# medical-genomics-group/VAMPomi

Measured on AMD Instinct MI355X. Metric: VAMP iterations/s (+ achieved HBM GB/s of the A/A^T kernels), higher is better.
Workload: dtype f64

## Files before the change

### include/vampomi.h

```cpp
#ifndef VAMPOMI_H
#define VAMPOMI_H

#include <stddef.h>
#include <stdint.h>

#ifdef __cplusplus
extern "C" {
#endif

#define VAMPOMI_ABI_VERSION 3
#define VAMPOMI_MAX_L 64
#define VAMPOMI_MAX_C 64
#define VAMPOMI_MAX_SEGMENTS 64
#define VAMPOMI_UNIQUE_ID_BYTES 128

typedef enum {
    VAMPOMI_OK = 0,
    VAMPOMI_ERR_ARG = 1,
    VAMPOMI_ERR_HIP = 2,
    VAMPOMI_ERR_RCCL = 3,
    VAMPOMI_ERR_IO = 4,
    VAMPOMI_ERR_NAN_PHEN = 5,
    VAMPOMI_ERR_STATE = 6,
    VAMPOMI_ERR_OOM = 7,
// ... 171 lines not shown
    double bytes_total;
    double flops_total;
    int64_t timed;
    double ms_timed;
} vampomi_kernel_stat;

typedef struct {
    vampomi_kernel_stat ax;
    vampomi_kernel_stat atx;
    vampomi_kernel_stat ax_k[4];
    vampomi_kernel_stat atx_k[4];
    int64_t a_passes_exec;
    int64_t host_syncs;
    vampomi_kernel_stat loo;
    vampomi_kernel_stat op;
    vampomi_kernel_stat op_k[4];
    vampomi_kernel_stat coll;
} vampomi_stats;

vampomi_status vampomi_set_timing(vampomi_ctx* ctx, int on);
vampomi_status vampomi_get_stats(vampomi_ctx* ctx, vampomi_stats* out);
vampomi_status vampomi_reset_stats(vampomi_ctx* ctx);

vampomi_status vampomi_dev_set_variant(vampomi_ctx* ctx, int which, int variant);
vampomi_status vampomi_dev_prestep_counts(const vampomi_ctx* ctx, int64_t* made, int64_t* used);
vampomi_status vampomi_dev_time_pass(vampomi_ctx* ctx, int which, int K, int reps, double* avg_ms);
vampomi_status vampomi_dev_read_ceiling(vampomi_ctx* ctx, int reps, double* us_med, double* bytes, int* variant);
vampomi_status vampomi_dev_kernel_name(const vampomi_ctx* ctx, int which, int K, int mode, char* out, int cap);
vampomi_status vampomi_dev_ax_plan(int64_t N, int64_t M, int cus, int variant, int K, int* T, int* TR, int* S,
                                   int* grid, int* nslots, char* name, int cap);
vampomi_status vampomi_dev_op_plan(int64_t N, int64_t M, int cus, int variant, int K, int* T, int* S, int* TR,
                                   int* grid, int64_t* nslots, char* name, int cap);
vampomi_status vampomi_dev_op_lds(int64_t N, int64_t M, int cus, int variant, int K, int64_t* out);
vampomi_status vampomi_dev_op_timestamps(vampomi_ctx* ctx, unsigned long long* out, int cap, int* n);
vampomi_status vampomi_dev_mem_plan(int64_t N, int64_t Mt, int nranks, int rank, int cus, int probit, int writer,
                                    int64_t* bytes);
vampomi_status vampomi_dev_mem_plan_storage(int64_t N, int64_t Mt, int nranks, int rank, int cus, int probit,
                                            int writer, int storage, int64_t* bytes);
vampomi_status vampomi_dev_op_apply(vampomi_ctx* ctx, int K, const double* ar, const double* qo, const double* p,
                                    const double* z, const double* beta, double diag, double tau, double gam2,
                                    double* d, double* ad, double* dp);

#ifdef __cplusplus
}
#endif
#endif
```

### vampomi_amd/__init__.py

```python
from __future__ import annotations

import ctypes as C
from dataclasses import dataclass, field
from typing import Optional, Sequence

import numpy as np

from ._lib import (CLI_PATH, GEN_GAUSS, GEN_METH, LIB_PATH, MAX_L, MEM_DEVICE, MEM_HOST, NA_FATAL, NA_MEAN, NA_PASS,
                   STORE_F32, STORE_F64, STORE_U16, UNIQUE_ID_BYTES, Params, Result, ShardDesc, Stats, VampomiError,
                   check, load)

__all__ = ["Data", "Vamp", "VampOptions", "divide_work", "comm_unique_id", "phen_rows", "phen_rows_common", "read_labels", "adjust_basis", "VampomiError", "LIB_PATH", "CLI_PATH",
           "GEN_GAUSS", "GEN_METH", "STORE_F64", "STORE_F32", "STORE_U16", "load"]

_STORAGE = {"f64": STORE_F64, "f32": STORE_F32, "u16": STORE_U16}
_METH_NA = {"pass": NA_PASS, "fatal": NA_FATAL, "mean": NA_MEAN}


def _dp(a: np.ndarray):
    return a.ctypes.data_as(C.c_void_p)


def divide_work(Mt: int, nranks: int, rank: int):
    M, S, Mm = C.c_int64(), C.c_int64(), C.c_int64()
# ... 416 lines not shown
        pr = np.ascontiguousarray(probs, dtype=np.float64)
        va = np.ascontiguousarray(vars_scaled, dtype=np.float64)
        x1 = np.zeros(max(self.M, 1))
        x1d = np.zeros(max(self.M, 1))
        s = C.c_double()
        check(self._lib.vampomi_denoise(self.ctx, _dp(r1), gam1, _dp(pr), _dp(va), L, _dp(x1), _dp(x1d),
                                        C.byref(s), MEM_HOST))
        return x1[: self.M], x1d[: self.M], s.value

    def kernel_name(self, which: int, K: int, mode: int = 0) -> str:
        buf = C.create_string_buffer(256)
        check(self._lib.vampomi_dev_kernel_name(self.ctx, which, K, mode, buf, 256))
        return buf.value.decode()

    def op_apply(self, ar, p, diag: float, tau: float, gam2: float, z=None, qo=None, beta=None):
        ar = np.ascontiguousarray(np.atleast_2d(ar), dtype=np.float64)
        p = np.ascontiguousarray(np.atleast_2d(p), dtype=np.float64)
        K = ar.shape[0]
        if ar.shape != (K, self.N) or p.shape != (K, self.M):
            raise ValueError("ar must be K x N and p K x M")
        fz = z is not None
        if fz:
            z = np.ascontiguousarray(np.atleast_2d(z), dtype=np.float64)
            qo = np.ascontiguousarray(np.atleast_2d(qo), dtype=np.float64)
            beta = np.ascontiguousarray(beta, dtype=np.float64)
        d = np.zeros((K, max(self.M, 1)))
        ad = np.zeros((K, self.N))
        dp = np.zeros(K)
        check(self._lib.vampomi_dev_op_apply(self.ctx, K, _dp(ar), _dp(qo) if fz else None, _dp(p),
                                             _dp(z) if fz else None, _dp(beta) if fz else None, diag, tau, gam2,
                                             _dp(d), _dp(ad), _dp(dp)))
        return d[:, : self.M], ad, dp

    def read_ceiling(self, reps: int = 9) -> dict:
        us, nb, var = C.c_double(), C.c_double(), C.c_int()
        check(self._lib.vampomi_dev_read_ceiling(self.ctx, int(reps), C.byref(us), C.byref(nb), C.byref(var)))
        return {"us_med": us.value, "bytes": nb.value, "GBs": nb.value / (us.value * 1e-6) / 1e9,
                "variant": ("lockstep 8-wave workgroups, one per CU", "1 MiB chunk per wave")[var.value]}

    def set_variant(self, which: int, variant: int):
        check(self._lib.vampomi_dev_set_variant(self.ctx, which, variant))

    def prestep_counts(self) -> tuple:
        made, used = C.c_int64(), C.c_int64()
        check(self._lib.vampomi_dev_prestep_counts(self.ctx, C.byref(made), C.byref(used)))
        return made.value, used.value

    def all_ok(self, local_ok: bool) -> bool:
        out = C.c_int()
        check(self._lib.vampomi_all_ok(self.ctx, 1 if local_ok else 0, C.byref(out)))
        return bool(out.value)

    def comm_abort(self):
        check(self._lib.vampomi_comm_abort(self.ctx))

    def set_timing(self, on: bool = True, period: int = 1):
        check(self._lib.vampomi_set_timing(self.ctx, (max(1, int(period)) if on else 0)))

    def stats(self) -> Stats:
        s = Stats()
        check(self._lib.vampomi_get_stats(self.ctx, C.byref(s)))
        return s

    def reset_stats(self):
        check(self._lib.vampomi_reset_stats(self.ctx))

# ... 146 lines not shown
```

### vampomi_amd/_lib.py

```python
from __future__ import annotations

import ctypes as C
import os

try:
    import torch
except Exception:
    torch = None

HERE = os.path.dirname(os.path.abspath(__file__))
LIB_PATH = os.environ.get("VAMPOMI_LIB") or os.path.join(HERE, "lib", "libvampomi.so")
CLI_PATH = os.path.join(HERE, "bin", "main_meth.exe")

MAX_L = 64
MAX_C = 64
UNIQUE_ID_BYTES = 128
MEM_HOST, MEM_DEVICE = 0, 1
GEN_GAUSS, GEN_METH = 0, 1
STORE_F64, STORE_F32, STORE_U16 = 0, 1, 16
NA_PASS, NA_FATAL, NA_MEAN = 0, 1, 2

STATUS = {
    0: "OK", 1: "ERR_ARG", 2: "ERR_HIP", 3: "ERR_RCCL", 4: "ERR_IO",
    5: "ERR_NAN_PHEN", 6: "ERR_STATE", 7: "ERR_OOM", 8: "ERR_MODEL",
# ... 121 lines not shown
    "vampomi_read_covariates": (C.c_int, [_P, C.c_char_p, C.c_int]),
    "vampomi_set_covariates": (C.c_int, [_P, _P, C.c_int, C.c_int64, C.c_int]),
    "vampomi_get_covariates": (C.c_int, [_P, _P]),
    "vampomi_cov_eval": (C.c_int, [_P, _P, _P, _P, _P, C.POINTER(C.c_double), C.c_int]),
    "vampomi_newton_cov": (C.c_int, [_P, _P, _P, _P, C.POINTER(C.c_int), _P, _P, C.c_int]),
    "vampomi_get_cov_eff": (C.c_int, [_P, _P]),
    "vampomi_get_probit_state": (C.c_int, [_P, _P, C.POINTER(C.c_double)]),
    "vampomi_denoise": (C.c_int, [_P, _P, C.c_double, _P, _P, C.c_int, _P, _P, C.POINTER(C.c_double), C.c_int]),
    "vampomi_params_default": (None, [C.POINTER(Params)]),
    "vampomi_infere": (C.c_int, [_P, C.POINTER(Params), C.POINTER(Result)]),
    "vampomi_vamp_begin": (C.c_int, [_P, C.POINTER(Params), C.POINTER(Result)]),
    "vampomi_vamp_step": (C.c_int, [_P, C.POINTER(C.c_int)]),
    "vampomi_step_phases": (C.c_int, [_P, C.POINTER(C.c_double), C.POINTER(C.c_double)]),
    "vampomi_vamp_end": (C.c_int, [_P]),
    "vampomi_set_timing": (C.c_int, [_P, C.c_int]),
    "vampomi_get_stats": (C.c_int, [_P, C.POINTER(Stats)]),
    "vampomi_reset_stats": (C.c_int, [_P]),
    "vampomi_dev_set_variant": (C.c_int, [_P, C.c_int, C.c_int]),
    "vampomi_dev_prestep_counts": (C.c_int, [_P, C.POINTER(C.c_int64), C.POINTER(C.c_int64)]),
    "vampomi_dev_time_pass": (C.c_int, [_P, C.c_int, C.c_int, C.c_int, C.POINTER(C.c_double)]),
    "vampomi_dev_read_ceiling": (C.c_int, [_P, C.c_int, C.POINTER(C.c_double), C.POINTER(C.c_double),
                                           C.POINTER(C.c_int)]),
    "vampomi_dev_kernel_name": (C.c_int, [_P, C.c_int, C.c_int, C.c_int, C.c_char_p, C.c_int]),
    "vampomi_dev_mem_plan": (C.c_int, [C.c_int64, C.c_int64, C.c_int, C.c_int, C.c_int, C.c_int, C.c_int, _P]),
    "vampomi_dev_mem_plan_storage": (C.c_int, [C.c_int64, C.c_int64, C.c_int, C.c_int, C.c_int, C.c_int, C.c_int,
                                               C.c_int, _P]),
    "vampomi_dev_ax_plan": (C.c_int, [C.c_int64, C.c_int64, C.c_int, C.c_int, C.c_int, _P, _P, _P, _P, _P, C.c_char_p,
                                      C.c_int]),
    "vampomi_dev_op_plan": (C.c_int, [C.c_int64, C.c_int64, C.c_int, C.c_int, C.c_int, _P, _P, _P, _P, _P, C.c_char_p,
                                      C.c_int]),
    "vampomi_dev_op_lds": (C.c_int, [C.c_int64, C.c_int64, C.c_int, C.c_int, C.c_int, _P]),
    "vampomi_dev_op_apply": (C.c_int, [_P, C.c_int, _P, _P, _P, _P, _P, C.c_double, C.c_double, C.c_double, _P, _P,
                                       _P]),
    "vampomi_dev_op_timestamps": (C.c_int, [_P, _P, C.c_int, C.POINTER(C.c_int)]),
    "vampomi_all_ok": (C.c_int, [_P, C.c_int, C.POINTER(C.c_int)]),
    "vampomi_comm_abort": (C.c_int, [_P]),
}

_lib = None


def load() -> C.CDLL:
    global _lib
    if _lib is None:
        if not os.path.exists(LIB_PATH):
            raise ImportError(f"{LIB_PATH} not built: run `python -m vampomi_amd.build`")
        lib = C.CDLL(LIB_PATH, mode=C.RTLD_GLOBAL)
        other = bool(os.environ.get("VAMPOMI_LIB"))
        for name, (res, args) in SIGNATURES.items():
            if other and not hasattr(lib, name):
                continue
            f = getattr(lib, name)
            f.restype = res
            f.argtypes = args
        _lib = lib
    return _lib


def check(status: int) -> None:
    if status != 0:
        msg = load().vampomi_last_error()
        raise VampomiError(status, msg.decode() if msg else "")
```

### vampomi_amd/csrc/atax_team.hip

```cpp
#include <hip/hip_ext.h>

#include <algorithm>
#include <cstdio>
#include <mutex>
#include <string>
#include <type_traits>

#include "kdev.h"

namespace vk {

typedef unsigned int v4u __attribute__((ext_vector_type(4)));
typedef unsigned int v2u __attribute__((ext_vector_type(2)));

#ifndef TM_FMA
#define TM_FMA 1
#endif
#ifndef TM_SAFE
#define TM_SAFE 0
#endif
#ifndef TM_TS
#define TM_TS 0
#endif
#ifndef TM_TEAMS_BY_XCD
// ... 143 lines not shown
__device__ __forceinline__ XE tm_ld1(__amdgpu_buffer_rsrc_t rs, int off) {
    if constexpr (sizeof(XE) == 8)
        return __builtin_bit_cast(double, __builtin_amdgcn_raw_buffer_load_b64(rs, off, 0, 2));
    else if constexpr (sizeof(XE) == 4)
        return __builtin_bit_cast(float, __builtin_amdgcn_raw_buffer_load_b32(rs, off, 0, 2));
    else
        return (uint16_t)__builtin_amdgcn_raw_buffer_load_b16(rs, off, 0, 2);
}

template <class Tp>
__device__ __forceinline__ Tp* tm_chk(Tp* p, const void* lo, const void* hi, unsigned code, unsigned* err) {
#if TM_SAFE
    if ((const char*)p < (const char*)lo || (const char*)p >= (const char*)hi) {
        __hip_atomic_fetch_or(err, 1u | (code << 1), __ATOMIC_RELAXED, __HIP_MEMORY_SCOPE_SYSTEM);
        return (Tp*)lo;
    }
#endif
    return p;
}

template <int K>
struct TmSlots {
    const double* ar[K];
    const double* p[K];
    double* d[K];
    double* sraw[K];
    double diag[K], tau[K], gam2[K];
};
template <int K>
__device__ __forceinline__ TmSlots<K> tm_slots(const OpArgs& a, int alt) {
    TmSlots<K> s;
#pragma unroll
    for (int k = 0; k < K; ++k) {
        int idx = k == alt ? kOpMaxK : k;
        asm volatile("" : "+s"(idx));
        const OpAlt::Slot& t = a.alt.tab[idx];
        s.ar[k] = t.ar;
        s.p[k] = t.p;
        s.d[k] = t.d;
        s.sraw[k] = t.sraw;
        s.diag[k] = t.diag;
        s.tau[k] = t.tau;
        s.gam2[k] = t.gam2;
    }
    return s;
}

template <int K, int S, int F, int L, int P, bool COMM, int E, bool FMA, int KP, class XE>
__device__ __forceinline__ void atax_team_body(const XE* __restrict__ X, int64_t ld, int64_t N, int64_t M,
                                               const double* __restrict__ mave, const double* __restrict__ msig,
                                               const OpArgs& a, int T, int TR, int ilv,
                                               const int* __restrict__ gate) {
    extern __shared__ __attribute__((aligned(16))) double lds[];
    double* s_beta = lds;
    if (a.fold.on) {
        double& s_go = lds[kOpMaxK];
        if (threadIdx.x == 0) {
            CgState cs = *a.fold.src;
            double r[3 * kMaxRhs];
#pragma unroll
            for (int q = 0; q < 3 * kMaxRhs; ++q) r[q] = q < 3 * cs.K ? a.fold.red[q] : 0.0;
            const bool ran = cg_decide_into(cs, r, a.fold.it, a.fold.mask);
            if (blockIdx.x == 0) {
                *a.fold.dst = cs;
                cg_publish(cs, ran, a.fold.it, a.fold.mirror, a.fold.flag, a.fold.seq, a.fold.pack);
            }
            s_go = cs.any ? 1.0 : 0.0;
#pragma unroll
            for (int k = 0; k < kOpMaxK; ++k) s_beta[k] = cs.beta[k];
        }
        __syncthreads();
        if (s_go == 0.0) return;
    } else if (gate && !*gate) {
        return;
    }
    const double* beta = a.fold.on ? s_beta : a.beta;
    static_assert(K + KP <= kMaxRhs, "partial slots per team");
    int fuse = a.fuse, alt = -1;
    if constexpr (KP == 0) {
        if (a.alt.cs && !a.fold.on) alt = cg_pre_slot(a.alt.cs->active, K, *a.alt.done == a.alt.token);
        if (alt >= 0) fuse &= ~(1 << alt);
    }
#if TM_TS
    const unsigned long long ts0 = __builtin_amdgcn_s_memrealtime();
#endif
    const int dbg = TM_ABL ? TM_ABL : (TM_DBG || !COMM) ? a.dbg : 0;
    constexpr int CW = COMM ? 7 : 8;
    constexpr int RS = tm_rows_per_step(COMM, E);
    static_assert(E == 1 || E == 2, "doubles per lane per load");
    constexpr int RING = F + L + 1;
    static_assert(COMM || L == 0, "without a hand-off the column is finished in its own step");
    static_assert(!COMM || (P >= 1 && P <= L), "polls in flight");
    static_assert(!COMM || P < RING, "a poll's slot is consumed before it is reissued");
    const int wave = threadIdx.x >> 6, lane = threadIdx.x & 63;
    const int g = blockIdx.x >> 3;
    const int member = g % T;
    const int nteams = gridDim.x / T;
#if TM_TEAMS_BY_XCD
    const int team = g / T + (nteams >> 3) * (int)(blockIdx.x & 7);
#else
    const int team = (blockIdx.x & 7) + 8 * (g / T);
#endif
    const int64_t cs = ilv ? nteams : 1;
    const int64_t mb = ilv ? team : (int64_t)team * M / nteams;
    const int n = (int)(ilv ? (M - team + nteams - 1) / nteams : (int64_t)(team + 1) * M / nteams - mb);
    const int64_t nmax = (M + nteams - 1) / nteams;
    const int64_t gwords = (M + gridDim.x) * kOpMaxK * T * 2;
    const int64_t r0 = (int64_t)member * TR;
    const int nrows = (int)(N - r0 < TR ? N - r0 : TR);
    constexpr bool QFULL = tm_qfull(K, S, COMM, E);
    const TmLds lay = tm_lds(K, S, COMM, E, TR < N ? TR : N);
    const int QS = (int)lay.qs;
    double* q_lds = lds + lay.q;
    double* s_part = lds + lay.part;
    double* s_tot = lds + lay.tot;
    const int jb = 64 * E * wave + E * lane;
    constexpr int XB = (int)sizeof(XE);
    const int nbytes = (E == 2 ? (nrows + 1) & ~1 : nrows) * XB;

    if (COMM && wave == CW) {
        const TmSlots<K> sl = tm_slots<K>(a, alt);
        const int nq = K * T;
        unsigned long long* xg = a.xg + (int64_t)team * nmax * nq * 2;
        unsigned long long* dummy = a.xg + gwords + (int64_t)blockIdx.x * 2 * K;
        const bool qv = (lane >> 5) < K && (lane & 31) < T;
        const int ql2 = qv ? 2 * ((lane >> 5) * T + (lane & 31)) : 0;
        const int nq2 = 2 * nq;
        const int csi = (int)cs;
        const unsigned tag = a.tag;
        const double* scp = msig;
#pragma unroll
        for (int k = 0; k < K; ++k) {
            if (lane == 1 + k) scp = sl.p[k];
            if (lane == 1 + K + k && ((fuse >> k) & 1)) scp = a.z.p[k];
        }
        scp += mb;
        double bk[K], dpacc[K];
#pragma unroll
        for (int k = 0; k < K; ++k) {
            bk[k] = ((fuse >> k) & 1) ? beta[k] : 0.0;
            dpacc[k] = 0.0;
        }
        v4u pl[RING];
        v2u ps[RING];
        bool dead = false;
        unsigned nslow = 0, nspin = 0;
        if (n > 0) {
            bool l2 = false;
            {
                unsigned long long* hdr = a.xg + gwords + (int64_t)gridDim.x * 2 * kOpMaxK + (int64_t)team * T;
                unsigned xcc;
                asm volatile("s_getreg_b32 %0, hwreg(HW_REG_XCC_ID)" : "=s"(xcc));
                xcc &= 0xf;
                if (lane == 0)
                    __hip_atomic_store(hdr + member, ((unsigned long long)tag << 32) | xcc, __ATOMIC_RELAXED,
                                       __HIP_MEMORY_SCOPE_AGENT);
                unsigned long long h = 0;
                for (unsigned spins = 0;; ++spins) {
                    h = lane < T ? __hip_atomic_load(hdr + lane, __ATOMIC_RELAXED, __HIP_MEMORY_SCOPE_AGENT)
                                 : ((unsigned long long)tag << 32) | xcc;
                    if (__all((unsigned)(h >> 32) == tag)) break;
                    if (spins >= kTmMaxSpins) {
                        dead = true;
                        if (lane == 0) __hip_atomic_store(a.err, 1u, __ATOMIC_RELAXED, __HIP_MEMORY_SCOPE_SYSTEM);
                        break;
                    }
                    __builtin_amdgcn_s_sleep(2);
                }
                l2 = !dead && __all((unsigned)h == xcc);
                if (dbg & 32) l2 = false;
            }
            for (int base = -F; base - L < n; base += RING) {
#pragma unroll
                for (int i = 0; i < RING; ++i) {
                    const int m = base + i;
                    if (dbg & 4096) {
                        __syncthreads();
                        continue;
                    }
                    const int ci = m - L + P, cf = m - L;
                    const int cic = ci < 0 ? 0 : ci < n ? ci : n - 1;
                    tm_load8(ps[(i + RING - L + P) % RING], scp + cic * csi);
                    tm_poll(pl[(i + RING - L + P) % RING], xg + (cic * nq2 + ql2));
                    v4u& g = pl[(i + RING - L) % RING];
                    v2u& sc = ps[(i + RING - L) % RING];
                    if (!(dbg & 1)) tm_wait2<3 * P>(g, sc);
                    if (cf >= 0 && cf < n) {
                        if (!(__all(g.y == tag && g.w == tag) || dead || (dbg & 1))) {
#pragma unroll 1
                            for (unsigned spins = 0;; ++spins) {
                                if (dbg & 64) {
                                    nslow += spins == 0;
                                    nspin++;
                                }
                                if (spins >= kTmMaxSpins) {
                                    dead = true;
                                    if (lane == 0) __hip_atomic_store(a.err, 1u, __ATOMIC_RELAXED, __HIP_MEMORY_SCOPE_SYSTEM);
                                    break;
                                }
                                __builtin_amdgcn_s_sleep(2);
                                tm_poll(g, tm_chk(xg + ((int64_t)cf * nq2 + ql2), a.xg, a.xg + gwords, 64, a.err));
                                tm_wait<0>(g);
                                if (__all(g.y == tag && g.w == tag)) break;
                            }
                        }
                        double v = qv ? __builtin_bit_cast(double, ((unsigned long long)g.z << 32) | g.x) : 0.0;
                        if (dbg & 512) {
                            for (int o = T >> 1; o > 0; o >>= 1) v += __shfl_xor(v, o, 64);
                        } else if (!(dbg & 256)) {
                            v = group_sum<32>(v);
                        }
                        const double scv = __builtin_bit_cast(double, ((unsigned long long)sc.y << 32) | sc.x);
                        const double sg = readlane_d(scv, 0);
                        const bool own = (cf & (T - 1)) == member;
                        const int64_t mg = mb + cf * csi;
                        double tsc[K], dval[K], pdir[K];
#pragma unroll
                        for (int k = 0; k < K; ++k) {
                            double t = sg * readlane_d(v, 32 * k);
                            t *= a.scale;
                            double p = readlane_d(scv, 1 + k);
                            if ((fuse >> k) & 1) p = readlane_d(scv, 1 + K + k) + bk[k] * p;
                            double val = t * sl.tau[k];
                            val += sl.gam2[k] * p;
                            tsc[k] = t;
                            dval[k] = val;
                            pdir[k] = p;
                        }
#pragma unroll
                        for (int k = 0; k < K; ++k)
                            if (lane == 0) s_tot[(cf & 1) * K + k] = (dbg & 128) ? 0.0 : sg * dval[k];
                        if (own) {
#pragma unroll
                            for (int k = 0; k < K; ++k) {
                                if (lane == 0 && !(dbg & 1024)) {
                                    if (a.sraw.p[0]) sl.sraw[k][mg] = tsc[k];
                                    *tm_chk(sl.d[k] + mg, sl.d[k], sl.d[k] + M, 128, a.err) = dval[k];
                                }
                                dpacc[k] += dval[k] * pdir[k];
                            }
                        }
                    }
                    __syncthreads();
                    if (lane < K && !(dbg & 2)) {
                        const bool real = m >= 0 && m < n;
                        double v = 0.0;
                        if (real) v = tree_sum<CW>(s_part + (m & 1) * CW * K + lane, K);
                        const unsigned long long u = __builtin_bit_cast(unsigned long long, v);
                        const v4u gr = {(unsigned)u, tag, (unsigned)(u >> 32), tag};
                        unsigned long long* dst =
                            tm_chk(real ? xg + ((int64_t)m * nq2 + (lane * T + member) * 2) : dummy + 2 * lane, a.xg,
                                   a.xg + gwords + (int64_t)gridDim.x * 2 * kOpMaxK, 512, a.err);
                        if (l2)
                            tm_publish_l2(dst, gr);
                        else
                            tm_publish(dst, gr);
                    }
                }
            }
#pragma unroll
            for (int s = 0; s < RING; ++s) tm_wait2<0>(pl[s], ps[s]);
            if ((dbg & 64) && lane == 0) {
                __hip_atomic_fetch_add(a.err + 1, nslow, __ATOMIC_RELAXED, __HIP_MEMORY_SCOPE_SYSTEM);
                __hip_atomic_fetch_add(a.err + 2, nspin, __ATOMIC_RELAXED, __HIP_MEMORY_SCOPE_SYSTEM);
                __hip_atomic_fetch_add(a.err + 3, (unsigned)n, __ATOMIC_RELAXED, __HIP_MEMORY_SCOPE_SYSTEM);
            }
        }
        if (lane == 0) {
#pragma unroll
            for (int k = 0; k < K; ++k) red_put(a.ro, (int64_t)blockIdx.x * K + k, dpacc[k]);
        }
        asm volatile("s_waitcnt vmcnt(0)" ::: "memory");
        __syncthreads();
        return;
    }

    const TmSlots<K> sl = tm_slots<K>(a, alt);
#pragma unroll
    for (int s = 0; s < S; ++s) {
        const int jl = RS * s + jb;
        if (jl >= QS) continue;
#pragma unroll
        for (int k = 0; k < K; ++k) {
#pragma unroll
            for (int h = 0; h < E; ++h) {
                double q = 0.0;
                if (jl + h < nrows) {
                    const int64_t j = r0 + jl + h;
                    q = sl.ar[k][j] / sl.diag[k];
                    if ((fuse >> k) & 1) q = q + beta[k] * a.qo.p[k][j];
                }
                q_lds[k * QS + jl + h] = q;
            }
        }
    }
    double bk[K];
#pragma unroll
    for (int k = 0; k < K; ++k) bk[k] = ((fuse >> k) & 1) ? beta[k] : 0.0;
    const double* pkp = mave;
    if (lane == 1) pkp = msig;
#pragma unroll
    for (int k = 0; k < K; ++k) {
        if (lane == 2 + k) pkp = sl.p[k];
        if (lane == 2 + K + k && ((fuse >> k) & 1)) pkp = a.z.p[k];
    }
#pragma unroll
    for (int k = 0; k < KP; ++k)
        if (lane == 2 + 2 * K + k) pkp = a.px.p[k];
    pkp += mb;
    bool valid[S];
#pragma unroll
    for (int s = 0; s < S; ++s) valid[s] = RS * s + jb < nrows;
    double acc[K][S][E];
#pragma unroll
    for (int k = 0; k < K; ++k)
#pragma unroll
        for (int s = 0; s < S; ++s)
#pragma unroll
            for (int e = 0; e < E; ++e) acc[k][s][e] = 0.0;
    double dpacc[K];
#pragma unroll
    for (int k = 0; k < K; ++k) dpacc[k] = 0.0;
    constexpr int KPA = KP > 0 ? KP : 1;
    double accp[KPA][S][E];
#pragma unroll
    for (int k = 0; k < KPA; ++k)
#pragma unroll
        for (int s = 0; s < S; ++s)
#pragma unroll
            for (int e = 0; e < E; ++e) accp[k][s][e] = 0.0;

    constexpr bool NW = XB < 8;
    typedef typename std::conditional<NW, XE, float>::type XW;
    double xr[NW ? 1 : RING][S][E];
    XW xw[NW ? RING : 1][S][E];
    double pk[RING];
    const char* xtile = reinterpret_cast<const char*>(X + mb * ld + r0);
// ... 46 lines not shown
            }
            if constexpr (KP > 0) {
#pragma unroll
                for (int k = 0; k < KP; ++k)
#pragma unroll
                    for (int e = 0; e < E; ++e) {
                        if constexpr (FMA)
                            accp[k][s][e] = __builtin_fma(dx[e], cp[k], accp[k][s][e]);
                        else
                            accp[k][s][e] += dx[e] * cp[k];
                    }
            }
#pragma unroll
            for (int k = 0; k < K; ++k) {
                if ((TM_DBG || TM_ABL) && (dbg & 2048)) {
                    q[k][0] = 0.5;
                    q[k][E - 1] = 0.25;
                } else if constexpr (E == 2) {
                    const v2d qq = *reinterpret_cast<const v2d*>(q_lds + k * QS + jq);
                    q[k][0] = qq.x;
                    q[k][E - 1] = qq.y;
                } else {
                    q[k][0] = q_lds[k * QS + jq];
                }
#pragma unroll
                for (int e = 0; e < E; ++e) {
                    if constexpr (FMA)
                        v[k] = __builtin_fma(dx[e], q[k][e], v[k]);
                    else
                        v[k] += dx[e] * q[k][e];
                }
            }
        }
        if (K == 2) {
            double r0, r1;
            swap32(v[0], v[K - 1], r0, r1);
            double keep = r0 + r1;
            if (dbg & 512) {
                for (int o = 16; o > 0; o >>= 1) keep += __shfl_xor(keep, o, 64);
            } else if (!(dbg & 4)) {
                keep = group_sum<32>(keep);
            }
            if ((lane & 31) == 0) s_part[(par * CW + wave) * K + (lane >> 5)] = keep;
        } else {
            if (!(dbg & 4)) v[0] = group_sum<64>(v[0]);
            if (lane == 0) s_part[(par * CW + wave) * K] = v[0];
        }
    };
    auto finish = [&](int slot, int m, const double (&tot)[K]) {
        double cc[K];
        if constexpr (COMM) {
#pragma unroll
            for (int k = 0; k < K; ++k) cc[k] = tot[k];
        } else {
            const double sg = readlane_d(pk[slot], 1);
            const bool own = (m % T) == member;
            const int64_t mg = mb + m * cs;
#pragma unroll
            for (int k = 0; k < K; ++k) {
                double t = sg * tot[k];
                t *= a.scale;
                double p = readlane_d(pk[slot], 2 + k);
                if ((fuse >> k) & 1) p = readlane_d(pk[slot], 2 + K + k) + bk[k] * p;
                double val = t * sl.tau[k];
                val += sl.gam2[k] * p;
                if (own) {
                    if (threadIdx.x == 0) {
                        if (a.sraw.p[0]) sl.sraw[k][mg] = t;
                        sl.d[k][mg] = val;
                    }
                    dpacc[k] += val * p;
                }
                cc[k] = sg * val;
            }
        }
        const double mu = NW ? readlane_d(pk[slot], 0) : 0.0;
#pragma unroll
        for (int s = 0; s < S; ++s) {
            if (dbg & 8) break;
            const double me_ = QFULL || valid[s] ? mu : 0.0;
#pragma unroll
            for (int k = 0; k < K; ++k)
#pragma unroll
                for (int e = 0; e < E; ++e) {
                    double dx;
                    if constexpr (NW)
                        dx = widen1(xw[slot][s][e]) - me_;
                    else
                        dx = xr[slot][s][e];
                    if constexpr (FMA)
                        acc[k][s][e] = __builtin_fma(dx, cc[k], acc[k][s][e]);
                    else
                        acc[k][s][e] += dx * cc[k];
                }
        }
    };
// ... 18 lines not shown
                            double t = 0.0;
#pragma unroll
                            for (int w = 0; w < CW; ++w) t += s_part[((m & 1) * CW + w) * K + k];
                            tot[k] = t;
                        }
                    }
                    finish((i + RING - L) % RING, cf, tot);
                }
            }
        }
    }
    double* dst = a.part + (int64_t)team * kMaxRhs * ld + r0;
#pragma unroll
    for (int s = 0; s < S; ++s) {
        const int jl = RS * s + jb;
        if (jl >= nrows) continue;
#pragma unroll
        for (int k = 0; k < K; ++k)
#pragma unroll
            for (int e = 0; e < E; ++e)
                if (jl + e < nrows) dst[(int64_t)k * ld + jl + e] = acc[k][s][e];
        if constexpr (KP > 0) {
#pragma unroll
            for (int k = 0; k < KP; ++k)
#pragma unroll
                for (int e = 0; e < E; ++e)
                    if (jl + e < nrows) dst[(int64_t)(K + k) * ld + jl + e] = accp[k][s][e];
        }
    }
    if constexpr (COMM) {
        __syncthreads();
    } else if (threadIdx.x == 0) {
#pragma unroll
        for (int k = 0; k < K; ++k) red_put(a.ro, (int64_t)blockIdx.x * K + k, dpacc[k]);
    }
    if (wave == 0) ticket_sum_blocks<K>(a.ro);
#if TM_TS
    if (a.ts && threadIdx.x == 0) {
        unsigned xcc, hw;
        asm volatile("s_getreg_b32 %0, hwreg(HW_REG_XCC_ID)" : "=s"(xcc));
        asm volatile("s_getreg_b32 %0, hwreg(HW_REG_HW_ID)" : "=s"(hw));
        unsigned long long* t = a.ts + 4 * (int64_t)blockIdx.x;
        t[0] = ts0;
        t[1] = __builtin_amdgcn_s_memrealtime();
        t[2] = xcc;
        t[3] = hw;
    }
#endif
}

template <int K, int S, int F, int L, int P, bool COMM, int E, bool FMA>
__global__ __launch_bounds__(kTmThreads) void atax_team_kernel(const double* __restrict__ X, int64_t ld, int64_t N,
                                                               int64_t M, const double* __restrict__ mave,
                                                               const double* __restrict__ msig, OpArgs a, int T,
                                                               int TR, int ilv, const int* __restrict__ gate) {
    atax_team_body<K, S, F, L, P, COMM, E, FMA, 0>(X, ld, N, M, mave, msig, a, T, TR, ilv, gate);
}

template <int K, int S, int F, int L, int P, bool COMM, int E, bool FMA>
__global__ __launch_bounds__(kTmThreads) void atax_team_kernel_f32(const float* __restrict__ X, int64_t ld,
                                                                   int64_t N, int64_t M,
                                                                   const double* __restrict__ mave,
                                                                   const double* __restrict__ msig, OpArgs a, int T,
                                                                   int TR, int ilv, const int* __restrict__ gate) {
    atax_team_body<K, S, F, L, P, COMM, E, FMA, 0>(X, ld, N, M, mave, msig, a, T, TR, ilv, gate);
}

template <int K, int S, int F, int L, int P, bool COMM, int E, bool FMA>
__global__ __launch_bounds__(kTmThreads) void atax_team_kernel_u16(const uint16_t* __restrict__ X, int64_t ld,
// ... 167 lines not shown
static int tm_S(int64_t rows, bool comm, int E) {
    const int rs = tm_rows_per_step(comm, E);
    return (int)((rows + rs - 1) / rs);
}

bool team_plan(int64_t N, int64_t M, int cus, int T, int cfg, OpPlan* out) {
    if (cfg < 0 || cfg >= kTmNCfg || N < 1) return false;
    const TmCfg& c = kTmCfg[cfg];
    if ((T == 1) == c.comm) return false;
    if (T < 1 || T > kTmMaxT || (T & (T - 1))) return false;
    const int grid = (cus / (8 * T)) * 8 * T;
    if (grid < T) return false;
    int64_t TR = N;
    if (T > 1) {
        TR = c.E == 2 ? ((N + T - 1) / T + 127) / 128 * 128 : (N + T - 1) / T;
        if ((int64_t)(T - 1) * TR >= N) return false;
    }
    const int S = tm_S(TR, c.comm, c.E);
    if (S > c.maxS) return false;
    for (int K = 1; K <= kOpMaxK; ++K)
        if (tm_lds(K, S, c.comm, c.E, std::min<int64_t>(TR, N)).words * 8 > kTmLdsMaxBytes) return false;
    OpPlan p{};
    p.grid = grid;
    p.S = S;
    p.T = T;
    p.TR = (int)TR;
    p.cfg = cfg;
    p.nslots = grid / T;
    (void)M;
    *out = p;
    return true;
}

bool team_lds_layout(const OpPlan& pl, int64_t N, int K, int64_t out[6]) {
    if (pl.T < 1 || pl.cfg < 0 || pl.cfg >= kTmNCfg || K < 1 || K > kOpMaxK || N < 1) return false;
    const TmCfg& c = kTmCfg[pl.cfg];
    const TmLds l = tm_lds(K, pl.S, c.comm, c.E, std::min<int64_t>(pl.TR, N));
    out[0] = kTmLdsHead;
    out[1] = l.q;
    out[2] = l.qs;
    out[3] = l.part;
    out[4] = l.tot;
    out[5] = l.words;
    return true;
}

template <int K, int S, int C, bool PL, class XE>
static hipError_t launch_tm_e(const Shard& s, const OpPlan& pl, const OpArgs& a, hipStream_t st, const Timing& tm,
                              const int* gate, int* occ) {
    constexpr TmCfg c = kTmCfg[C];
    static_assert(!PL || K == 1, "the head-start kernel has one operator system");
    constexpr bool F32 = sizeof(XE) == 4, U16 = sizeof(XE) == 2;
    void (*kern)(const XE*, int64_t, int64_t, int64_t, const double*, const double*, OpArgs, int, int, int,
                 const int*);
    if constexpr (PL && U16)
        kern = atax_team_plain_kernel_u16<S, c.F, c.L, c.P, c.comm, c.E, (bool)TM_FMA>;
    else if constexpr (U16)
        kern = atax_team_kernel_u16<K, S, c.F, c.L, c.P, c.comm, c.E, (bool)TM_FMA>;
    else if constexpr (PL && F32)
        kern = atax_team_plain_kernel_f32<S, c.F, c.L, c.P, c.comm, c.E, (bool)TM_FMA>;
    else if constexpr (PL)
        kern = atax_team_plain_kernel<S, c.F, c.L, c.P, c.comm, c.E, (bool)TM_FMA>;
    else if constexpr (F32)
        kern = atax_team_kernel_f32<K, S, c.F, c.L, c.P, c.comm, c.E, (bool)TM_FMA>;
    else
        kern = atax_team_kernel<K, S, c.F, c.L, c.P, c.comm, c.E, (bool)TM_FMA>;
    const size_t lds = (size_t)tm_lds(K, S, c.comm, c.E, std::min<int64_t>(pl.TR, s.N)).words * sizeof(double);
    if (lds > (size_t)kTmLdsMaxBytes) return hipErrorInvalidValue;
    static std::atomic<unsigned long long> allowed{0};
    if (const hipError_t e = lds_allow(reinterpret_cast<const void*>(kern), allowed, (int)kTmLdsMaxBytes))
        return e;
    if (occ) {
        if (hipOccupancyMaxActiveBlocksPerMultiprocessor(occ, kern, kTmThreads, lds) != hipSuccess) *occ = 0;
        return hipSuccess;
    }
    hipExtLaunchKernelGGL(kern, dim3(pl.grid), dim3(kTmThreads), lds, st, tm.start, tm.stop, 0,
                          static_cast<const XE*>(s.X), s.ld, s.N, s.M, s.mave, s.msig, a, pl.T, pl.TR, c.ilv ? 1 : 0,
                          gate);
    return hipSuccess;
}

template <int K, int S, int C, bool PL>
static hipError_t launch_tm(const Shard& s, const OpPlan& pl, const OpArgs& a, hipStream_t st, const Timing& tm,
                            const int* gate, int* occ) {
    if (s.u16) return launch_tm_e<K, S, C, PL, uint16_t>(s, pl, a, st, tm, gate, occ);
    if (s.f32) return launch_tm_e<K, S, C, PL, float>(s, pl, a, st, tm, gate, occ);
    return launch_tm_e<K, S, C, PL, double>(s, pl, a, st, tm, gate, occ);
}

static constexpr int tm_plain_maxS(int cfg) {
    return cfg == 0 ? 8 : cfg == 2 ? 3 : cfg == 3 ? 4 : cfg == 4 ? 5 : 0;
}

template <int K, int C, int S, bool PL>
static hipError_t launch_tm_if(const Shard& s, const OpPlan& pl, const OpArgs& a, hipStream_t st, const Timing& tm,
                               const int* gate, int* occ) {
    if constexpr (S <= (PL ? tm_plain_maxS(C) : kTmCfg[C].maxS))
        return launch_tm<K, S, C, PL>(s, pl, a, st, tm, gate, occ);
    return hipErrorInvalidValue;
}

template <int K, int C, bool PL>
static hipError_t launch_tm_s(int S, const Shard& s, const OpPlan& pl, const OpArgs& a, hipStream_t st,
                        const Timing& tm, const int* gate, int* occ) {
    switch (S) {
        case 1: return launch_tm_if<K, C, 1, PL>(s, pl, a, st, tm, gate, occ);
        case 2: return launch_tm_if<K, C, 2, PL>(s, pl, a, st, tm, gate, occ);
        case 3: return launch_tm_if<K, C, 3, PL>(s, pl, a, st, tm, gate, occ);
        case 4: return launch_tm_if<K, C, 4, PL>(s, pl, a, st, tm, gate, occ);
        case 5: return launch_tm_if<K, C, 5, PL>(s, pl, a, st, tm, gate, occ);
        case 6: return launch_tm_if<K, C, 6, PL>(s, pl, a, st, tm, gate, occ);
        case 7: return launch_tm_if<K, C, 7, PL>(s, pl, a, st, tm, gate, occ);
        case 8: return launch_tm_if<K, C, 8, PL>(s, pl, a, st, tm, gate, occ);
        case 9: return launch_tm_if<K, C, 9, PL>(s, pl, a, st, tm, gate, occ);
        case 10: return launch_tm_if<K, C, 10, PL>(s, pl, a, st, tm, gate, occ);
        default: return hipErrorInvalidValue;
    }
}

static OpArgs tm_with_slots(const OpArgs& a, int K) {
    OpArgs x = a;
    for (int k = 0; k < K && k < kOpMaxK; ++k)
        x.alt.tab[k] = OpAlt::Slot{a.ar.p[k], a.p.p[k], a.d.p[k], a.sraw.p[k], a.diag, a.tau, a.gam2};
    x.alt.tab[kOpMaxK] = OpAlt::Slot{a.alt.ar, a.alt.p, a.alt.d, a.sraw.p[0] ? a.alt.d : nullptr, 1.0, 1.0, 0.0};
    return x;
}

template <int K, bool PL = false>
static hipError_t launch_tm_c(const Shard& s, const OpPlan& pl, const OpArgs& a0, hipStream_t st, const Timing& tm,
                        const int* gate, int* occ = nullptr) {
    const OpArgs a = tm_with_slots(a0, K);
    if constexpr (PL) {
        switch (pl.cfg) {
            case 0: return launch_tm_s<1, 0, true>(pl.S, s, pl, a, st, tm, gate, occ);
            case 2: return launch_tm_s<1, 2, true>(pl.S, s, pl, a, st, tm, gate, occ);
            case 3: return launch_tm_s<1, 3, true>(pl.S, s, pl, a, st, tm, gate, occ);
            case 4: return launch_tm_s<1, 4, true>(pl.S, s, pl, a, st, tm, gate, occ);
            default: return hipErrorInvalidValue;
        }
    }
    switch (pl.cfg) {
        case 0: return launch_tm_s<K, 0, false>(pl.S, s, pl, a, st, tm, gate, occ);
        case 1: return launch_tm_s<K, 1, false>(pl.S, s, pl, a, st, tm, gate, occ);
        case 2: return launch_tm_s<K, 2, false>(pl.S, s, pl, a, st, tm, gate, occ);
        case 3: return launch_tm_s<K, 3, false>(pl.S, s, pl, a, st, tm, gate, occ);
        case 4: return launch_tm_s<K, 4, false>(pl.S, s, pl, a, st, tm, gate, occ);
        case 5: return launch_tm_s<K, 5, false>(pl.S, s, pl, a, st, tm, gate, occ);
        case 6: return launch_tm_s<K, 6, false>(pl.S, s, pl, a, st, tm, gate, occ);
        default: return hipErrorInvalidValue;
    }
}

hipError_t atax_team(const Shard& s, const OpPlan& pl, int K, const OpArgs& a, hipStream_t st, const Timing& tm,
                     const int* gate) {
    if (pl.T < 1 || pl.grid < pl.T || pl.grid % pl.T) return hipErrorInvalidValue;
    if (pl.T > 1 && (!a.xg || !a.err || a.tag == 0)) return hipErrorInvalidValue;
    if (s.M <= 0) return hipSuccess;
    hipError_t e = hipErrorInvalidValue;
    switch (K) {
        case 1: e = launch_tm_c<1>(s, pl, a, st, tm, gate); break;
        case 2: e = launch_tm_c<2>(s, pl, a, st, tm, gate); break;
        default: break;
    }
    if (e != hipSuccess) return e;
    return hipGetLastError();
}

hipError_t atax_team_plain(const Shard& s, const OpPlan& pl, const OpArgs& a, hipStream_t st, const Timing& tm,
                           const int* gate) {
    if (pl.T < 1 || pl.grid < pl.T || pl.grid % pl.T) return hipErrorInvalidValue;
    if (pl.T > 1 && (!a.xg || !a.err || a.tag == 0)) return hipErrorInvalidValue;
    for (int k = 0; k < kTmPlain; ++k)
        if (!a.px.p[k]) return hipErrorInvalidValue;
    if (s.M <= 0) return hipSuccess;
    if (const hipError_t e = launch_tm_c<1, true>(s, pl, a, st, tm, gate)) return e;
    return hipGetLastError();
}

bool ax_team_plan(int64_t N, int64_t M, int cus, AxPlan* out) {
    if (N < 1 || cus < 8) return false;
    constexpr int RS = tm_rows_per_step(false, 2);
    for (int T = 1; T <= kTmMaxT; T *= 2) {
        if (cus / (8 * T) < 1) break;
        const int grid = (cus / (8 * T)) * 8 * T;
        const int64_t TR = T == 1 ? N : ((N + T - 1) / T + 127) / 128 * 128;
        if ((int64_t)(T - 1) * TR >= N) continue;
        const int S = (int)((TR + RS - 1) / RS);
        if (S > kAxTmMaxS) continue;
        AxPlan p{};
        p.variant = kAxTeam;
        p.T = T;
        p.TR = (int)TR;
        p.S = S;
        p.groups = grid;
// ... 54 lines not shown
}

std::string ax_kernel_name(int K, bool fused, const AxPlan& pl, int ek) {
    if (pl.T <= 0) return kernel_name(0, K, fused ? 1 : 0, pl.variant, ek);
    char b[96];
    std::snprintf(b, sizeof b, "ax_team_kernel%s<%d, %d, %s>", xe_suffix(ek), pl.S, K, fused ? "true" : "false");
    return b;
}

bool team_plain_plan(int64_t N, int64_t M, int cus, const OpPlan& main, OpPlan* out) {
    const int cfgs1[] = {0};
    const int cfgsT[] = {2, 3, 4};
    for (int T = std::max(main.T, 1); T <= kTmMaxT; T *= 2) {
        const int* cf = T == 1 ? cfgs1 : cfgsT;
        const int ncf = T == 1 ? 1 : 3;
        for (int i = 0; i < ncf; ++i) {
            OpPlan p{};
            if (!team_plan(N, M, cus, T, cf[i], &p) || p.S > tm_plain_maxS(cf[i])) continue;
            *out = p;
            return true;
        }
    }
    return false;
}

int team_occupancy(const OpPlan& pl, int K, int ek) {
    int occ = 0;
    const Shard s{nullptr, 0, (int64_t)pl.TR * pl.T, 1, nullptr, nullptr, ek == kXF32, ek == kXU16};
    const OpArgs a{};
    hipError_t e = hipErrorInvalidValue;
    switch (K) {
        case 1: e = launch_tm_c<1>(s, pl, a, nullptr, Timing{}, nullptr, &occ); break;
        case 2: e = launch_tm_c<2>(s, pl, a, nullptr, Timing{}, nullptr, &occ); break;
        case 1 + kTmPlain: e = launch_tm_c<1, true>(s, pl, a, nullptr, Timing{}, nullptr, &occ); break;
        default: break;
    }
    return e == hipSuccess ? occ : 0;
}

std::string team_kernel_name(int K, const OpPlan& pl, int ek) {
    const TmCfg& c = kTmCfg[pl.cfg];
    const char* sfx = xe_suffix(ek);
    char b[128];
    if (K == 1 + kTmPlain)
        std::snprintf(b, sizeof b, "atax_team_plain_kernel%s<%d, %d, %d, %d, %s, %d>", sfx, pl.S, c.F, c.L, c.P,
                      c.comm ? "true" : "false", c.E);
    else
        std::snprintf(b, sizeof b, "atax_team_kernel%s<%d, %d, %d, %d, %d, %s, %d>", sfx, K, pl.S, c.F, c.L, c.P,
                      c.comm ? "true" : "false", c.E);
    return b;
}

}
```

### vampomi_amd/csrc/ctx.h

```cpp
#pragma once
#include <hip/hip_runtime.h>
#include <rccl/rccl.h>

#include <cstdint>
#include <initializer_list>
#include <memory>
#include <string>
#include <utility>
#include <vector>

#include "../../include/vampomi.h"
#include "kernels.h"

vampomi_status fail(vampomi_status s, const std::string& msg);

#define HIPCHK(expr)                                                                                  \
    do {                                                                                              \
        hipError_t _e = (expr);                                                                       \
        if (_e != hipSuccess)                                                                         \
            return fail(VAMPOMI_ERR_HIP, std::string(#expr) + ": " + hipGetErrorString(_e));          \
    } while (0)

#define NCCLCHK(expr)                                                                                 \
    do {                                                                                              \
// ... 89 lines not shown
    int atx_variant = vk::kAtxDefault, loo_variant = vk::kLooDefault;
    double* ax_part = nullptr;
    double* red_part = nullptr;
    size_t red_cap = 0;
    double* scal = nullptr;
    double* h_scal = nullptr;
    double* d_hscal = nullptr;
    unsigned* ticket = nullptr;
    unsigned long long* h_flag = nullptr;
    unsigned long long* d_flag = nullptr;
    unsigned long long sync_seq = 0;
    vk::CgState* cgs = nullptr;
    vk::CgMirror* h_cgm = nullptr;
    vk::CgMirror* d_cgm = nullptr;
    vk::OpPlan opp{};
    int op_variant = vk::kOpDefault;
    bool op_ready = false;
    bool op_ok_mine = false;
    bool op_ok = false;
    bool op_agreed = false;
    int op_variant_req = vk::kOpDefault;
    int cus = 0;
    double* op_part = nullptr;
    int64_t op_part_slots = 0;
    double* op_nvec = nullptr;
    unsigned long long* op_xg = nullptr;
    size_t op_xg_words = 0;
    unsigned op_tag = 0;
    vk::OpPlan opp_hs{};
    bool hs_ok_mine = false;
    bool hs_ok = false;
    bool hs_on = true;
    bool hs_on_req = true;
    int pre_mode = 2;
    unsigned long long pre_seq = 0;
    int64_t pre_made_n = 0, pre_used_n = 0;
    unsigned long long* op_ts = nullptr;
    double* nbuf = nullptr;
    double* mbuf = nullptr;
    double* am_n = nullptr;
    double* am_m = nullptr;
    double* lc_z = nullptr;
    double* lc_part = nullptr;
    int32_t* lc_idx = nullptr;
    int lc_G = 0;
    int64_t lc_slots = 0, lc_idx_cap = 0;

    bool timing = false;
    int tperiod = 1;
    int64_t tcount[5][vk::kMaxRhs] = {};
    std::vector<TimedLaunch> pending;
    std::vector<hipEvent_t> ev_pool;
    vampomi_stats stats{};

    std::unique_ptr<VampRun> run;
    std::unique_ptr<IterWriter> writer;

    bool f32() const { return storage == VAMPOMI_STORE_F32; }
    bool u16() const { return storage == VAMPOMI_STORE_U16; }
    int ek() const { return u16() ? vk::kXU16 : f32() ? vk::kXF32 : vk::kXF64; }
    int64_t esize() const { return u16() ? 2 : f32() ? 4 : 8; }
    vk::Shard shard() const { return vk::Shard{X, ld, N, M, mave, msig, f32() ? 1 : 0, u16() ? 1 : 0}; }
    vampomi_ctx();
    ~vampomi_ctx();
};

// ... 62 lines not shown
    vampomi_ctx* c_;
    int nsync_ = 0, nlocal_ = 0;
    int nred_ = 0;
    unsigned long long last_seq_ = 0;
    std::vector<Sink> sinks_;
};

inline vk::DotTerm T(const double* a, const double* b, int op = vk::DOT) { return vk::DotTerm{a, b, op}; }

struct CgSystem {
    const double* v = nullptr;
    double* mu = nullptr;
    bool mu0_nonzero = false;
    const double* atx0 = nullptr;
    double* W = nullptr;
    double* S = nullptr;
    double* AW = nullptr;
    bool onsager = false;
    int iters = 0;
    double *r = nullptr, *z = nullptr, *p = nullptr, *d = nullptr;
};
struct HeadStart {
    double* abern = nullptr;
    const double* xnext = nullptr;
    double* axnext = nullptr;
    bool used = false;
    double* T1 = nullptr;
    double* U1 = nullptr;
    unsigned long long* pre_done = nullptr;
    bool pre_have = false;
    bool pre_offer = false;
    bool pre_made = false;
    bool pre_used = false;
};
enum class PreMode { normal, ahead, queued };
struct PcgArgs {
    double tau = 0.0, gam2 = 0.0;
    int max_iter = 0;
    double tol = 0.0;
    double* nscratch = nullptr;
    int64_t* ref_passes = nullptr;
    DotBatch* init = nullptr;
    const double* extra_x = nullptr;
    double* ex_out = nullptr;
    bool onepass = false;
    const double* const* ar0 = nullptr;
    HeadStart* hs = nullptr;
    const vk::Prelude* pre = nullptr;
    PreMode pm = PreMode::normal;
};
vampomi_status pcg_run(vampomi_ctx* c, const std::vector<CgSystem*>& sys, const PcgArgs& args);
vampomi_status op_prepare(vampomi_ctx* c);
vampomi_status op_agree(vampomi_ctx* c);
vampomi_status headstart_available(vampomi_ctx* c, bool* yes);
constexpr int64_t kPreMinBytes = (int64_t)256 << 20;
bool prestep_on(const vampomi_ctx* c);
unsigned* op_err_dev(vampomi_ctx* c);
vampomi_status op_check_err(vampomi_ctx* c);
vampomi_status op_dev(vampomi_ctx* c, int K, const vk::OpArgs& a, const int* gate, bool reduce = true,
                      bool divide = true);
vampomi_status op_dev_plain(vampomi_ctx* c, const vk::OpArgs& a, const double* const* px, double* const* out,
                            const int* gate);

vampomi_status cov_eval_dev(vampomi_ctx* c, const double* gg, const double* eta, double* H, double* rhs,
                            double* mlogL);
vampomi_status cov_newton_dev(vampomi_ctx* c, const double* gg, const double* eta0, double* eta, int* iters,
                              int* backtracks, double* rel_err);
vampomi_status cov_offset_dev(vampomi_ctx* c, const double* eta, double* m);
```

### vampomi_amd/csrc/engine.cpp

```cpp
#include <hip/hip_runtime.h>
#include <rccl/rccl.h>

#include <algorithm>
#include <cfloat>
#include <chrono>
#include <condition_variable>
#include <map>
#include <mutex>
#include <cmath>
#include <cstdio>
#include <cstdlib>
#include <cstring>
#include <memory>
#include <string>
#include <thread>
#include <vector>

#include "ctx.h"
#include "hostio.h"
#include "writer.h"

static thread_local std::string g_err;
static thread_local vampomi_ctx* g_coll_ctx = nullptr;

// ... 618 lines not shown
                              const double* const* zf, const double* beta, bool dp, double* const* sraw) {
    if (!c->have_X) return fail(VAMPOMI_ERR_STATE, "ATx before the methylation data was loaded");
    if (c->M <= 0) return VAMPOMI_OK;
    vk::CPtrs us{}, ps{}, zs{};
    vk::Ptrs os{}, ss{};
    for (int k = 0; k < K; ++k) {
        us.p[k] = u[k];
        os.p[k] = out[k];
        ss.p[k] = sraw ? sraw[k] : nullptr;
        ps.p[k] = p ? p[k] : nullptr;
        zs.p[k] = zf ? zf[k] : nullptr;
    }
    TimedLaunch t = launch_stat(c, 1, K, pass_bytes(c, K), pass_flops(c, K));
    HIPCHK(vk::atx(c->shard(), K, us, os, 1.0 / c->sqrtN, mode, tau, gam2, ps, c->st, c->atx_variant, vk::Timing{t.a, t.b}, gate, zs,
                   zf ? beta : nullptr, ss));
    c->stats.a_passes_exec++;
    if (mode == 1 && dp) {
        vk::DotArgs a{};
        a.nt = K;
        for (int k = 0; k < K; ++k)
            a.t[k] = zf ? vk::DotTerm{out[k], p[k], vk::PUPD, zf[k], beta + k} : vk::DotTerm{out[k], p[k], vk::DOT};
        HIPCHK(vk::dots(a, c->M, vk::RedOut{c->red_part, c->scal + SL_DP, c->ticket, nullptr, 0, gate}, c->st));
        STCHK(allreduce_dev(c, c->scal + SL_DP, K));
    }
    return VAMPOMI_OK;
}

static size_t red_capacity(int64_t Mx) {
    return std::max<size_t>({(size_t)vk::kRedBlocks * 3 * vk::kMaxRhs, (size_t)vk::kRedBlocks * vk::kMaxTerms,
                             (size_t)((Mx + 255) / 256) * (1 + 2 * (vk::kMaxL - 1)),
                             (size_t)(Mx / 8 + 1) * vk::kMaxRhs, (size_t)4096});
}

static size_t op_xg_words_for(int64_t Mx, const vk::OpPlan& p) {
    return (size_t)(Mx + p.grid) * vk::kOpMaxK * (size_t)p.T * 2 + (size_t)p.grid * (2 * vk::kOpMaxK + 1);
}

static vampomi_status op_plan_local(vampomi_ctx* c) {
    if (c->cus <= 0) HIPCHK(hipDeviceGetAttribute(&c->cus, hipDeviceAttributeMultiprocessorCount, c->device));
    const int64_t M = std::max<int64_t>(c->M, 1);
    bool op_ok = vk::op_plan(c->N, M, c->cus, c->op_variant, &c->opp);
    if (op_ok && c->opp.T >= 1) {
        for (int K = 1; K <= vk::kOpMaxK && op_ok; ++K) {
            const int occ = vk::team_occupancy(c->opp, K, c->ek());
            if ((int64_t)occ * c->cus < c->opp.grid) {
                std::fprintf(stderr, "libvampomi: one-pass operator off: %s fits %d workgroup(s) per CU; the plan "
                                     "needs %lld resident on %d CUs (two passes per CG step)\n",
                             vk::team_kernel_name(K, c->opp, c->ek()).c_str(), occ, (long long)c->opp.grid, c->cus);
                op_ok = false;
            }
        }
    }
    bool hs_ok = op_ok && vk::team_plain_plan(c->N, M, c->cus, c->opp, &c->opp_hs);
    if (hs_ok && (int64_t)vk::team_occupancy(c->opp_hs, 1 + vk::kOpPlain, c->ek()) * c->cus < c->opp_hs.grid) hs_ok = false;
    c->op_ok_mine = op_ok;
    c->hs_ok_mine = hs_ok;
    if (!c->op_ts && std::getenv("VAMPOMI_OP_TS") && std::atoi(std::getenv("VAMPOMI_OP_TS"))) {
        HIPCHK(hipMalloc((void**)&c->op_ts, (size_t)4 * 8 * std::max(c->cus, 1) * 2));
        HIPCHK(hipMemsetAsync(c->op_ts, 0, (size_t)4 * 8 * std::max(c->cus, 1) * 2, c->st));
    }
    if (!c->op_nvec) {
        STCHK(dev_alloc(&c->op_nvec, (size_t)3 * vk::kMaxRhs * c->ld + 16));
        HIPCHK(hipMemsetAsync(c->op_nvec, 0, ((size_t)3 * vk::kMaxRhs * c->ld + 16) * 8, c->st));
    }
    if (op_ok) {
        const int64_t slots = std::max<int64_t>(c->opp.nslots, hs_ok ? c->opp_hs.nslots : 0);
        if (slots > c->op_part_slots) {
            dev_free(c->op_part);
            STCHK(dev_alloc(&c->op_part, (size_t)slots * vk::kMaxRhs * c->ld));
            c->op_part_slots = slots;
        }
        if (c->opp.T > 1 || (hs_ok && c->opp_hs.T > 1)) {
            size_t words = c->opp.T > 1 ? op_xg_words_for(M, c->opp) : 0;
            if (hs_ok && c->opp_hs.T > 1) words = std::max(words, op_xg_words_for(M, c->opp_hs));
            if (words > c->op_xg_words) {
                if (c->op_xg) (void)hipFree(c->op_xg);
                c->op_xg = nullptr;
                c->op_xg_words = 0;
                HIPCHK(hipMalloc((void**)&c->op_xg, words * 8));
                HIPCHK(hipMemsetAsync(c->op_xg, 0, words * 8, c->st));
                c->op_xg_words = words;
            }
        }
    }
    c->op_ready = true;
    return VAMPOMI_OK;
}

vampomi_status op_prepare(vampomi_ctx* c) {
    if (!c->op_ready) STCHK(op_plan_local(c));
    if (!c->use_comm) {
        c->op_ok = c->op_ok_mine;
        c->hs_ok = c->hs_ok_mine && c->hs_on;
    } else if (!c->op_agreed) {
        c->op_ok = c->hs_ok = false;
    }
    return VAMPOMI_OK;
}

vampomi_status op_agree(vampomi_ctx* c) {
    if (!c->use_comm) return VAMPOMI_OK;
    if (c->op_variant_req != c->op_variant || c->hs_on_req != c->hs_on) {
        c->op_variant = c->op_variant_req;
        c->hs_on = c->hs_on_req;
        c->op_ready = false;
    }
    bool op = false, hs = false;
// ... 64 lines not shown
        HIPCHK(launch());
        return VAMPOMI_OK;
    }
    if (g.fence) {
        for (vampomi_ctx* o : g.ctxs) {
            if (o == c) continue;
            if (!o->team_ev) return fail(VAMPOMI_ERR_HIP, "team gate: no event for a context");
            HIPCHK(hipEventRecord(o->team_ev, o->st));
            HIPCHK(hipStreamWaitEvent(c->st, o->team_ev, 0));
        }
        g.fence = false;
    } else if (g.last) {
        HIPCHK(hipStreamWaitEvent(c->st, g.last, 0));
    }
    HIPCHK(launch());
    if (!g.last) HIPCHK(hipEventCreateWithFlags(&g.last, hipEventDisableTiming));
    HIPCHK(hipEventRecord(g.last, c->st));
    return VAMPOMI_OK;
}

vampomi_status op_check_err(vampomi_ctx* c) {
    const unsigned e = c->h_flag ? __atomic_exchange_n(reinterpret_cast<unsigned*>(c->h_flag + 4), 0u, __ATOMIC_ACQ_REL) : 0u;
    if (e > 1)
        return fail(VAMPOMI_ERR_HIP, "one-pass operator: address checks failed (codes " + std::to_string(e >> 1) + ")");
    if (e)
        return fail(VAMPOMI_ERR_HIP, "one-pass operator: a team hand-off timed out (a workgroup of the team never "
                                     "ran: fewer compute units than planned?)");
    return VAMPOMI_OK;
}

vampomi_status op_dev(vampomi_ctx* c, int K, const vk::OpArgs& a, const int* gate, bool reduce, bool divide) {
    if (!c->have_X) return fail(VAMPOMI_ERR_STATE, "A before the methylation data was loaded");
    STCHK(op_prepare(c));
    if (!c->op_ok || K < 1 || K > vk::kOpMaxK)
        return fail(VAMPOMI_ERR_ARG, "one-pass operator: K <= 2 and a plan for N = " + std::to_string(c->N));
    double* ad = c->op_nvec + (int64_t)2 * vk::kMaxRhs * c->ld;
    vk::OpArgs x = a;
    x.part = c->op_part;
    x.scale = 1.0 / c->sqrtN;
    if (c->opp.T > 1) {
        x.xg = c->op_xg;
        if (++c->op_tag == 0) ++c->op_tag;
        x.tag = c->op_tag;
        x.err = op_err_dev(c);
    }
    static const int dbg = std::getenv("VAMPOMI_OP_DBG") ? std::atoi(std::getenv("VAMPOMI_OP_DBG")) : 0;
    x.dbg = dbg;
    x.ts = c->op_ts;
    x.ro = vk::RedOut{c->red_part, c->use_comm ? ad + (int64_t)K * c->ld : c->scal + SL_DP, c->ticket, nullptr, 0,
                      gate};
    TimedLaunch t = launch_stat(c, 3, K, pass_bytes(c, K), 2.0 * pass_flops(c, K));
    STCHK(team_launch(c, c->opp.T,
                      [&] { return vk::atax(c->shard(), c->opp, K, x, c->st, vk::Timing{t.a, t.b}, gate); }));
    c->stats.a_passes_exec++;
    vk::Ptrs os{};
    for (int k = 0; k < K; ++k) os.p[k] = ad + (int64_t)k * c->ld;
    if (!c->use_comm) {
        if (reduce) HIPCHK(vk::op_reduce(c->opp, K, c->N, c->ld, c->op_part, os, c->sqrtN, c->st, gate));
    } else {
        HIPCHK(vk::op_reduce(c->opp, K, c->N, c->ld, c->op_part, os, 0.0, c->st, gate));
        STCHK(allreduce_dev(c, ad, (size_t)K * c->ld + K));
        if (divide) HIPCHK(vk::vec_div(K, c->N, c->ld, os, c->sqrtN, c->st));
    }
    return VAMPOMI_OK;
}

vampomi_status op_dev_plain(vampomi_ctx* c, const vk::OpArgs& a, const double* const* px, double* const* out,
                            const int* gate) {
    if (!c->have_X) return fail(VAMPOMI_ERR_STATE, "A before the methylation data was loaded");
    STCHK(op_prepare(c));
    if (!c->hs_ok) return fail(VAMPOMI_ERR_ARG, "head-start launch: no plan for N = " + std::to_string(c->N));
    constexpr int KT = 1 + vk::kOpPlain;
    double* ad = c->op_nvec + (int64_t)2 * vk::kMaxRhs * c->ld;
    vk::OpArgs x = a;
    x.part = c->op_part;
    x.scale = 1.0 / c->sqrtN;
    for (int k = 0; k < vk::kOpPlain; ++k) x.px.p[k] = px[k];
    if (c->opp_hs.T > 1) {
        x.xg = c->op_xg;
        if (++c->op_tag == 0) ++c->op_tag;
        x.tag = c->op_tag;
        x.err = op_err_dev(c);
    }
    x.dbg = 0;
    x.ro = vk::RedOut{c->red_part, c->use_comm ? ad + (int64_t)KT * c->ld : c->scal + SL_DP, c->ticket, nullptr, 0,
                      gate};
    TimedLaunch t = launch_stat(c, 3, KT, pass_bytes(c, KT), pass_flops(c, 1) + pass_flops(c, KT));
    STCHK(team_launch(c, c->opp_hs.T, [&] {
        return vk::atax_team_plain(c->shard(), c->opp_hs, x, c->st, vk::Timing{t.a, t.b}, gate);
    }));
    c->stats.a_passes_exec++;
// ... 143 lines not shown
    STCHK(dev_alloc(&c->msig, Mx));
    STCHK(dev_alloc(&c->y, c->ld));
    HIPCHK(hipMemsetAsync(c->y, 0, c->ld * 8, c->st));
    STCHK(dev_alloc(&c->ax_part, (size_t)c->axp.nslots * vk::kMaxRhs * c->ld));
    c->red_cap = red_capacity(Mx);
    STCHK(dev_alloc(&c->red_part, c->red_cap));
    c->writer.reset(new IterWriter());
    STCHK(c->writer->open(c.get()));
    STCHK(dev_alloc(&c->scal, SL_TOTAL));
    HIPCHK(hipHostMalloc((void**)&c->h_scal, SL_TOTAL * sizeof(double), hipHostMallocMapped | hipHostMallocCoherent));
    HIPCHK(hipHostGetDevicePointer((void**)&c->d_hscal, c->h_scal, 0));
    HIPCHK(hipHostMalloc((void**)&c->h_flag, 64, hipHostMallocMapped | hipHostMallocCoherent));
    std::memset(c->h_flag, 0, 64);
    HIPCHK(hipHostGetDevicePointer((void**)&c->d_flag, c->h_flag, 0));
    HIPCHK(hipMalloc((void**)&c->ticket, 64 * sizeof(unsigned)));
    HIPCHK(hipMemsetAsync(c->ticket, 0, 64 * sizeof(unsigned), c->st));
    STCHK(dev_alloc(&c->nbuf, (size_t)vk::kMaxRhs * c->ld));
    HIPCHK(hipMemsetAsync(c->nbuf, 0, (size_t)vk::kMaxRhs * c->ld * 8, c->st));
    STCHK(dev_alloc(&c->mbuf, (size_t)2 * vk::kMaxRhs * Mx));
    HIPCHK(hipMalloc((void**)&c->cgs, 2 * sizeof(vk::CgState)));
    HIPCHK(hipMemsetAsync(c->cgs, 0, 2 * sizeof(vk::CgState), c->st));
    HIPCHK(hipHostMalloc((void**)&c->h_cgm, vk::kCgMirrorSlots * sizeof(vk::CgMirror),
                         hipHostMallocMapped | hipHostMallocCoherent));
    std::memset(c->h_cgm, 0, vk::kCgMirrorSlots * sizeof(vk::CgMirror));
    HIPCHK(hipHostGetDevicePointer((void**)&c->d_cgm, c->h_cgm, 0));
    const char* force = std::getenv("VAMPOMI_FORCE_RCCL");
    c->use_comm = c->nranks > 1 || (force && std::atoi(force) != 0);
    if (const char* mv = std::getenv("VAMPOMI_MR_TAIL")) c->mr_tail = c->mr_tail_req = std::atoi(mv) != 0;
    if (const char* fv = std::getenv("VAMPOMI_CG_FOLD")) c->cg_fold = std::atoi(fv) != 0;
    if (const char* dv = std::getenv("VAMPOMI_DP_SEPARATE")) c->dp_separate = std::atoi(dv) != 0;
    if (const char* hv = std::getenv("VAMPOMI_HEADSTART")) c->hs_on = c->hs_on_req = std::atoi(hv) != 0;
    if (const char* pv = std::getenv("VAMPOMI_PRESTEP")) {
        const int v = std::atoi(pv);
        if (v >= 0 && v <= 2) c->pre_mode = v;
    }
    const char* mode = std::getenv("VAMPOMI_COMM");
    if (c->use_comm && mode && std::strcmp(mode, "loopback") == 0) {
        if (!d->comm_id) return fail(VAMPOMI_ERR_ARG, "the loopback communicator needs a communicator id");
        c->loopback = loopback_join(d->comm_id, c->nranks);
    } else if (c->use_comm && mode && std::strcmp(mode, "shm") == 0) {
        if (!d->comm_id) return fail(VAMPOMI_ERR_ARG, "the shm communicator needs a communicator id");
        std::string err;
        c->shm = shm_join(d->comm_id, c->nranks, c->rank, comm_init_timeout_s(), &err);
        if (!c->shm) return fail(VAMPOMI_ERR_STATE, err);
    } else if (c->use_comm) {
        ncclUniqueId id;
        if (d->comm_id)
            std::memcpy(&id, d->comm_id, sizeof id);
        else
            NCCLCHK(ncclGetUniqueId(&id));
        ncclConfig_t cfg = NCCL_CONFIG_INITIALIZER;
        cfg.blocking = 0;
        STCHK(nccl_settle(c.get(), ncclCommInitRankConfig(&c->comm, c->nranks, id, c->rank, &cfg),
                          "ncclCommInitRankConfig", comm_init_timeout_s()));
    }
    STCHK(sync_stream(c.get(), c->st));
    *out = c.release();
    return VAMPOMI_OK;
}

extern "C" vampomi_status vampomi_shard_info(const vampomi_ctx* c, int64_t* M, int64_t* S, int64_t* ld) {
    if (!c) return fail(VAMPOMI_ERR_ARG, "null context");
    if (M) *M = c->M;
    if (S) *S = c->S;
    if (ld) *ld = c->ld;
    return VAMPOMI_OK;
}
// ... 415 lines not shown
}

extern "C" vampomi_status vampomi_dev_set_variant(vampomi_ctx* c, int which, int variant) {
    if (!c) return fail(VAMPOMI_ERR_ARG, "null context");
    HIPCHK(hipSetDevice(c->device));
    STCHK(sync_stream(c, c->st));
    if (which == 0) {
        if (!vk::ax_variant_ok(variant)) return fail(VAMPOMI_ERR_ARG, "no such A.x variant");
        const vk::AxPlan np = vk::ax_plan(c->N, std::max<int64_t>(c->M, 1), variant);
        if (np.nslots > c->axp.nslots) {
            dev_free(c->ax_part);
            STCHK(dev_alloc(&c->ax_part, (size_t)np.nslots * vk::kMaxRhs * c->ld));
        }
        c->axp = np;
    } else if (which == 1) {
        if (!vk::atx_variant_ok(variant)) return fail(VAMPOMI_ERR_ARG, "no such A^T.u variant");
        c->atx_variant = variant;
    } else if (which == 3) {
        vk::OpPlan p{};
        if (!vk::op_plan(c->N, std::max<int64_t>(c->M, 1), c->cus > 0 ? c->cus : 256, variant, &p))
            return fail(VAMPOMI_ERR_ARG, "no such one-pass operator plan for this N");
        c->op_variant_req = variant;
        if (!c->use_comm) {
            c->op_variant = variant;
            c->op_ready = false;
        }
    } else if (which == 4) {
        return fail(VAMPOMI_ERR_ARG, "no side stream: every launch runs on the context's stream (DESIGN.md §6)");
    } else if (which == 5) {
        if (variant != 0 && variant != 1) return fail(VAMPOMI_ERR_ARG, "head start: 0 or 1");
        c->hs_on_req = variant == 1;
        if (!c->use_comm) c->hs_on = c->hs_on_req;
    } else if (which == 7) {
        if (variant < 0 || variant > 2) return fail(VAMPOMI_ERR_ARG, "pre-step: 0, 1 or 2");
        c->pre_mode = variant;
    } else if (which == 6) {
        if (variant != 0 && variant != 1) return fail(VAMPOMI_ERR_ARG, "multi-rank tail: 0 or 1");
        c->mr_tail_req = variant == 1;
        if (!c->use_comm) c->mr_tail = c->mr_tail_req;
    } else {
        if (!vk::loo_variant_ok(variant)) return fail(VAMPOMI_ERR_ARG, "no such association-pass variant");
        c->loo_variant = variant;
    }
    return VAMPOMI_OK;
}

bool prestep_on(const vampomi_ctx* c) {
    if (c->use_comm || c->nranks != 1 || !c->hs_ok || c->pre_mode == 0) return false;
    return c->pre_mode == 1 || std::max<int64_t>(c->M, 1) * c->ld * c->esize() >= kPreMinBytes;
}

extern "C" vampomi_status vampomi_dev_prestep_counts(const vampomi_ctx* c, int64_t* made, int64_t* used) {
    if (!c || !made || !used) return fail(VAMPOMI_ERR_ARG, "null argument");
    *made = c->pre_made_n;
    *used = c->pre_used_n;
    return VAMPOMI_OK;
}

extern "C" vampomi_status vampomi_dev_time_pass(vampomi_ctx* c, int which, int K, int reps, double* avg_ms) {
    if (!c || !avg_ms || K < 1 || K > (which == 0 ? 4 : which == 1 ? 3 : which == 3 ? 2 : 1) || reps < 1)
        return fail(VAMPOMI_ERR_ARG, "bad argument");
    if (!c->have_X) return fail(VAMPOMI_ERR_STATE, "no methylation data loaded");
    HIPCHK(hipSetDevice(c->device));
    if (which == 3) {
        STCHK(op_prepare(c));
        if (!c->op_ok_mine) return fail(VAMPOMI_ERR_ARG, "no one-pass operator plan for this N");
    }
    const int64_t Mx = std::max<int64_t>(c->M, 1);
    vk::CPtrs in{};
    vk::Ptrs out{};
    for (int k = 0; k < K; ++k) {
        in.p[k] = which == 0 ? c->mbuf + k * Mx : c->nbuf + k * c->ld;
        out.p[k] = which == 0 ? c->nbuf + k * c->ld : c->mbuf + k * Mx;
    }
    hipEvent_t a, b;
    HIPCHK(hipEventCreate(&a));
    HIPCHK(hipEventCreate(&b));
    HIPCHK(hipEventRecord(a, c->st));
    for (int r = 0; r < reps; ++r) {
        if (which == 0)
            HIPCHK(vk::ax_partial(c->shard(), c->axp, K, in, c->ax_part, c->st));
        else if (which == 1)
            HIPCHK(vk::atx(c->shard(), K, in, out, 1.0 / c->sqrtN, 0, 0.0, 0.0, vk::CPtrs{}, c->st, c->atx_variant));
        else if (which == 3) {
            vk::OpArgs x{};
            for (int k = 0; k < K; ++k) {
                x.ar.p[k] = c->nbuf + k * c->ld;
                x.p.p[k] = c->mbuf + k * Mx;
                x.d.p[k] = c->mbuf + (2 + k) * Mx;
            }
            x.diag = 1.0;
            x.scale = 1.0 / c->sqrtN;
            x.tau = 1.0;
            x.part = c->op_part;
            x.ro = vk::RedOut{c->red_part, c->scal + SL_DP, c->ticket, nullptr, 0, nullptr};
            if (c->opp.T > 1) {
                x.xg = c->op_xg;
                if (++c->op_tag == 0) ++c->op_tag;
                x.tag = c->op_tag;
                x.err = op_err_dev(c);
            }
            x.dbg = std::getenv("VAMPOMI_OP_DBG") ? std::atoi(std::getenv("VAMPOMI_OP_DBG")) : 0;
            if (c->opp.T > 1) x.err = op_err_dev(c);
            x.ts = c->op_ts;
            STCHK(team_launch(c, c->opp.T, [&] { return vk::atax(c->shard(), c->opp, K, x, c->st); }));
        }
        else
            HIPCHK(vk::loo_sums(c->shard(), c->nbuf, c->mbuf, c->sqrtN, c->mbuf + 3 * Mx, c->st, c->loo_variant));
    }
    HIPCHK(hipEventRecord(b, c->st));
    HIPCHK(hipEventSynchronize(b));
    if (which == 3 && std::getenv("VAMPOMI_OP_DBG") && (std::atoi(std::getenv("VAMPOMI_OP_DBG")) & 64)) {
        unsigned* w = reinterpret_cast<unsigned*>(c->h_flag + 4);
        std::fprintf(stderr, "op dbg: slow polls %u, spins %u, columns polled %u (over %d launches)\n", w[1], w[2], w[3],
                     reps);
        w[1] = w[2] = w[3] = 0;
    }
    float ms = 0.f;
    HIPCHK(hipEventElapsedTime(&ms, a, b));
    (void)hipEventDestroy(a);
    (void)hipEventDestroy(b);
    *avg_ms = (double)ms / reps;
    return VAMPOMI_OK;
}

extern "C" vampomi_status vampomi_dev_op_apply(vampomi_ctx* c, int K, const double* ar, const double* qo,
                                               const double* p, const double* z, const double* beta, double diag,
                                               double tau, double gam2, double* d, double* ad, double* dp) {
    if (!c || K < 1 || K > vk::kOpMaxK || !ar || !p || !d || !ad || !dp || (z && (!qo || !beta)))
        return fail(VAMPOMI_ERR_ARG, "bad argument");
    if (c->use_comm) return fail(VAMPOMI_ERR_ARG, "vampomi_dev_op_apply: one rank only");
    HIPCHK(hipSetDevice(c->device));
    STCHK(op_prepare(c));
    if (!c->op_ok) return fail(VAMPOMI_ERR_ARG, "no one-pass operator plan for this N");
    const int64_t Mx = std::max<int64_t>(c->M, 1);
    double* AR = c->op_nvec;
    double* Q = c->op_nvec + (int64_t)vk::kMaxRhs * c->ld;
    vk::OpArgs a{};
// ... 1 lines not shown
        STCHK(stage_in(c, ar + k * c->N, c->N, VAMPOMI_MEM_HOST, AR + k * c->ld));
        STCHK(stage_in(c, p + k * c->M, c->M, VAMPOMI_MEM_HOST, c->mbuf + k * Mx));
        a.ar.p[k] = AR + k * c->ld;
        a.p.p[k] = c->mbuf + k * Mx;
        a.d.p[k] = c->mbuf + (2 + k) * Mx;
        if (z) {
            STCHK(stage_in(c, qo + k * c->N, c->N, VAMPOMI_MEM_HOST, Q + k * c->ld));
            STCHK(stage_in(c, z + k * c->M, c->M, VAMPOMI_MEM_HOST, c->mbuf + (4 + k) * Mx));
            a.qo.p[k] = Q + k * c->ld;
            a.z.p[k] = c->mbuf + (4 + k) * Mx;
        }
    }
    double* dbeta = c->mbuf + 6 * Mx;
    if (z) {
        if (Mx < K) return fail(VAMPOMI_ERR_ARG, "vampomi_dev_op_apply: fused form needs M >= K");
        STCHK(stage_in(c, beta, K, VAMPOMI_MEM_HOST, dbeta));
        a.beta = dbeta;
        a.fuse = (1 << K) - 1;
    }
    a.diag = diag;
    a.tau = tau;
    a.gam2 = gam2;
    STCHK(op_dev(c, K, a, nullptr));
    const double* AD = c->op_nvec + (int64_t)2 * vk::kMaxRhs * c->ld;
    for (int k = 0; k < K; ++k) {
        STCHK(stage_out(c, c->mbuf + (2 + k) * Mx, c->M, VAMPOMI_MEM_HOST, d + k * c->M));
        STCHK(stage_out(c, AD + k * c->ld, c->N, VAMPOMI_MEM_HOST, ad + k * c->N));
    }
    HIPCHK(hipMemcpyAsync(dp, c->scal + SL_DP, (size_t)K * 8, hipMemcpyDeviceToHost, c->st));
    STCHK(sync_stream(c, c->st));
    return op_check_err(c);
}

extern "C" vampomi_status vampomi_dev_op_timestamps(vampomi_ctx* c, unsigned long long* out, int cap, int* n) {
    if (!c || !out || !n) return fail(VAMPOMI_ERR_ARG, "null argument");
    if (!c->op_ts) return fail(VAMPOMI_ERR_STATE, "no timestamps (VAMPOMI_OP_TS=1 at the first operator use)");
    STCHK(sync_stream(c, c->st));
    *n = std::min(cap, 4 * c->opp.grid);
    HIPCHK(hipMemcpy(out, c->op_ts, (size_t)*n * 8, hipMemcpyDeviceToHost));
    return VAMPOMI_OK;
}

extern "C" vampomi_status vampomi_dev_ax_plan(int64_t N, int64_t M, int cus, int variant, int K, int* T, int* TR,
                                              int* S, int* grid, int* nslots, char* name, int cap) {
    if (N < 1 || M < 1 || cus < 1 || K < 1 || K > vk::kMaxRhs || !vk::ax_variant_ok(variant))
        return fail(VAMPOMI_ERR_ARG, "bad argument");
    const vk::AxPlan p = vk::ax_plan_for(N, M, cus, variant);
    if (T) *T = p.T;
    if (TR) *TR = p.TR;
    if (S) *S = p.S;
    if (grid) *grid = p.groups;
    if (nslots) *nslots = p.nslots;
    if (name && cap > 0) std::snprintf(name, (size_t)cap, "%s", vk::ax_kernel_name(K, false, p).c_str());
    return VAMPOMI_OK;
}

extern "C" vampomi_status vampomi_dev_op_plan(int64_t N, int64_t M, int cus, int variant, int K, int* T, int* S,
                                              int* TR, int* grid, int64_t* nslots, char* name, int cap) {
    vk::OpPlan p{};
    if (K < 1 || K > vk::kOpMaxK || !vk::op_plan(N, std::max<int64_t>(M, 1), cus, variant, &p))
        return fail(VAMPOMI_ERR_ARG, "no one-pass operator plan");
    if (T) *T = p.T;
    if (S) *S = p.S;
    if (TR) *TR = p.TR;
    if (grid) *grid = p.grid;
    if (nslots) *nslots = p.nslots;
    if (name && cap > 0) std::snprintf(name, (size_t)cap, "%s", vk::op_kernel_name(K, p).c_str());
    return VAMPOMI_OK;
}

extern "C" vampomi_status vampomi_dev_op_lds(int64_t N, int64_t M, int cus, int variant, int K, int64_t* out) {
    vk::OpPlan p{};
    if (!out || !vk::op_plan(N, std::max<int64_t>(M, 1), cus, variant, &p) || !vk::team_lds_layout(p, N, K, out))
        return fail(VAMPOMI_ERR_ARG, "no team plan with that system count");
    return VAMPOMI_OK;
}

extern "C" vampomi_status vampomi_dev_mem_plan_storage(int64_t N, int64_t Mt, int nranks, int rank, int cus,
                                                       int probit, int writer, int storage, int64_t* bytes) {
    if (!bytes || N < 2 || Mt < nranks || nranks < 1 || rank < 0 || rank >= nranks || cus < 1 ||
        (storage != VAMPOMI_STORE_F64 && storage != VAMPOMI_STORE_F32 && storage != VAMPOMI_STORE_U16))
        return fail(VAMPOMI_ERR_ARG, "bad argument");
    int64_t M = 0, S = 0, Mm = 0;
    vampomi_divide_work(Mt, nranks, rank, &M, &S, &Mm);
    const int64_t Mx = std::max<int64_t>(M, 1), ld = (N + 15) / 16 * 16;
    int64_t total = 0;
    auto add = [&](int64_t n, int64_t elem) {
        const int64_t b = std::max<int64_t>(n, 1) * elem, g = 2 << 20;
        total += (b + g - 1) / g * g;
    };
    const vk::AxPlan axp = vk::ax_plan(N, Mx);
    add(Mx * ld, 8);
    add(Mx, 8), add(Mx, 8), add(ld, 8);
    add((int64_t)axp.nslots * vk::kMaxRhs * ld, 8);
    add((int64_t)red_capacity(Mx), 8), add((int64_t)red_capacity(Mx), 8);
    add(SL_TOTAL, 8), add(64, 4), add(64, 4);
    add((int64_t)vk::kMaxRhs * ld, 8);
    add((int64_t)2 * vk::kMaxRhs * Mx, 8);
    add((int64_t)sizeof(vk::CgState), 1);
    vk::OpPlan op{}, hs{};
    if (vk::op_plan(N, Mx, cus, vk::kOpDefault, &op)) {
        const bool h = vk::team_plain_plan(N, Mx, cus, op, &hs);
        add((int64_t)3 * vk::kMaxRhs * ld + 16, 8);
        add(std::max<int64_t>(op.nslots, h ? hs.nslots : 0) * vk::kMaxRhs * ld, 8);
        size_t w = op.T > 1 ? op_xg_words_for(Mx, op) : 0;
        if (h && hs.T > 1) w = std::max(w, op_xg_words_for(Mx, hs));
        if (w) add((int64_t)w, 8);
    }
    for (int q = 0; q < 25; ++q) add(Mx, 8);
    add(ld, 8), add((int64_t)vk::kMaxRhs * ld, 8), add((int64_t)vk::kMaxRhs * ld, 8), add(ld, 8);
    add(2 * ld, 8);
    add(Mx, 8), add(ld + 2, 8);
    if (probit) {
        for (int q = 0; q < 3; ++q) add(ld, 8);
        for (int q = 0; q < 3; ++q) add(Mx, 8);
    }
    (void)writer;
    if (storage == VAMPOMI_STORE_F32) total -= Mx * ld * 4;
    if (storage == VAMPOMI_STORE_U16) total -= Mx * ld * 6;
    *bytes = total;
    return VAMPOMI_OK;
}

extern "C" vampomi_status vampomi_dev_mem_plan(int64_t N, int64_t Mt, int nranks, int rank, int cus, int probit,
                                               int writer, int64_t* bytes) {
    return vampomi_dev_mem_plan_storage(N, Mt, nranks, rank, cus, probit, writer, VAMPOMI_STORE_F64, bytes);
}

static std::string op_name(const vampomi_ctx* c, int K) {
    vk::OpPlan p{};
    int cus = c->cus;
    if (cus <= 0 && hipDeviceGetAttribute(&cus, hipDeviceAttributeMultiprocessorCount, c->device) != hipSuccess) cus = 256;
    if (!vk::op_plan(c->N, std::max<int64_t>(c->M, 1), cus, c->op_variant, &p)) return "(no one-pass plan)";
    if (K == 1 + vk::kOpPlain) {
        vk::OpPlan h{};
        if (!vk::team_plain_plan(c->N, std::max<int64_t>(c->M, 1), cus, p, &h)) return "(no head-start plan)";
        return vk::team_kernel_name(K, h, c->ek());
    }
    return vk::op_kernel_name(K, p, c->ek());
}

extern "C" vampomi_status vampomi_dev_read_ceiling(vampomi_ctx* c, int reps, double* us_med, double* bytes,
                                                   int* variant) {
    if (!c || reps < 1 || !us_med) return fail(VAMPOMI_ERR_ARG, "bad argument");
    if (!c->have_X) return fail(VAMPOMI_ERR_STATE, "no methylation data loaded");
    HIPCHK(hipSetDevice(c->device));
    if (c->cus <= 0) HIPCHK(hipDeviceGetAttribute(&c->cus, hipDeviceAttributeMultiprocessorCount, c->device));
    STCHK(sync_stream(c, c->st));
    const int64_t n = std::max<int64_t>(c->M, 1) * c->ld;
    hipEvent_t a, b;
    HIPCHK(hipEventCreate(&a));
    HIPCHK(hipEventCreate(&b));
    double best = -1.0, best_bytes = 0.0;
    int best_kind = -1;
    for (int kind = 0; kind < 2; ++kind) {
        double nb = 0.0;
        if (vk::stream_read(c->X, c->ek(), n, kind, c->cus, c->st, vk::Timing{}, c->red_part, &nb) != hipSuccess) {
            (void)hipGetLastError();
            continue;
        }
        std::vector<float> ms((size_t)reps);
        for (int r = 0; r < reps; ++r) {
            HIPCHK(vk::stream_read(c->X, c->ek(), n, kind, c->cus, c->st, vk::Timing{a, b}, c->red_part, &nb));
            HIPCHK(hipEventSynchronize(b));
            HIPCHK(hipEventElapsedTime(&ms[(size_t)r], a, b));
        }
        std::sort(ms.begin(), ms.end());
        const double med = 1e3 * (double)ms[(size_t)reps / 2];
        if (best < 0.0 || nb / med > best_bytes / best) {
            best = med;
// ... 26 lines not shown
```

### vampomi_amd/csrc/kernels.h

```cpp
#pragma once
#include <hip/hip_runtime.h>

#include <atomic>
#include <cstdint>
#include <string>
#include <vector>

namespace vk {

constexpr int kMaxRhs = 4;
constexpr int kMaxL = 64;
constexpr int kMaxTerms = 12;
constexpr int kRedBlocks = 1024;

struct CPtrs { const double* p[kMaxRhs]; };
struct Timing { hipEvent_t start = nullptr, stop = nullptr; };
struct RedOut {
    double* part;
    double* out;
    unsigned* ticket;
    unsigned long long* flag = nullptr;
    unsigned long long seq = 0;
    const int* gate = nullptr;
    double* out2 = nullptr;
// ... 30 lines not shown
};
inline int64_t ax_slots(const AxPlan& p, int64_t t) { return ((t + 1) * p.sa - 1) / p.sb - (t * p.sa) / p.sb + 1; }
constexpr int kAxDefault = -1, kAxTeam = 7, kAxTeamMinT = 8, kAtxDefault = -1 , kLooDefault = 16;
AxPlan ax_plan(int64_t N, int64_t M, int variant = kAxDefault);
AxPlan ax_plan_for(int64_t N, int64_t M, int cus, int variant);
int ax_variant_count();
bool ax_variant_ok(int v);
int atx_variant_count();
bool atx_variant_ok(int v);
struct AxFuse {
    CPtrs z{};
    const double* beta = nullptr;
    const int* gate = nullptr;
};
hipError_t ax_partial(const Shard& s, const AxPlan& pl, int K, CPtrs x, double* part, hipStream_t st,
                      const Timing& tm = Timing{}, const AxFuse& fu = AxFuse{});
hipError_t stream_read(const void* x, int ek, int64_t n, int kind, int cus, hipStream_t st, const Timing& tm,
                       double* sink, double* bytes);
bool ax_team_plan(int64_t N, int64_t M, int cus, AxPlan* out);
hipError_t ax_team(const Shard& s, const AxPlan& pl, int K, CPtrs x, double* part, hipStream_t st, const Timing& tm,
                   const AxFuse& fu);
std::string ax_kernel_name(int K, bool fused, const AxPlan& pl, int ek = 0);
hipError_t ax_reduce(const AxPlan& pl, int K, int64_t N, int64_t ld, const double* part, Ptrs out,
                     double div, hipStream_t st, const int* gate = nullptr);
hipError_t vec_div(int K, int64_t n, int64_t ld, Ptrs v, double div, hipStream_t st, const Ptrs* dst = nullptr);

int atx_blocks(int64_t M, int K, int variant);
std::string kernel_name(int which, int K, int mode, int variant, int ek = 0);
hipError_t atx(const Shard& s, int K, CPtrs u, Ptrs out, double scale, int mode, double tau,
               double gam2, CPtrs p, hipStream_t st, int variant = kAtxDefault, const Timing& tm = Timing{},
               const int* gate = nullptr, CPtrs zf = CPtrs{}, const double* beta = nullptr, Ptrs sraw = Ptrs{});

constexpr int kOpMaxK = 2;
constexpr int kOpPlain = 3;
struct OpPlan {
    int grid;
    int S;
    int64_t nslots;
    int T = 0;
    int TR = 0;
    int cfg = 0;
};
constexpr int kOpDefault = -1;
bool op_plan(int64_t N, int64_t M, int cus, int variant, OpPlan* out);
bool op_supported(int64_t N, int K);
bool team_plan(int64_t N, int64_t M, int cus, int T, int cfg, OpPlan* out);
bool team_lds_layout(const OpPlan& pl, int64_t N, int K, int64_t out[6]);
hipError_t lds_allow(const void* kern, std::atomic<unsigned long long>& done, int bytes);
struct CgState;
struct CgMirror;
struct OpFold {
    const CgState* src = nullptr;
    CgState* dst = nullptr;
    const double* red = nullptr;
    int on = 0, it = 0, mask = 0xf, pack = 0;
    CgMirror* mirror = nullptr;
    unsigned long long* flag = nullptr;
    unsigned long long seq = 0;
};
struct OpAlt {
    const CgState* cs = nullptr;
    const unsigned long long* done = nullptr;
    unsigned long long token = 0;
    const double* ar = nullptr;
    const double* p = nullptr;
    double* d = nullptr;
// ... 5 lines not shown
        double diag, tau, gam2;
    };
    Slot tab[2 + 1];
};
struct OpArgs {
    CPtrs ar, qo;
    CPtrs p, z;
    const double* beta;
    int fuse;
    double diag, scale, tau, gam2;
    Ptrs d, sraw;
    CPtrs px;
    double* part;
    RedOut ro;
    unsigned long long* xg;
    unsigned tag;
    unsigned* err;
    unsigned long long* ts;
    int dbg;
    OpFold fold;
    OpAlt alt;
};
static_assert(sizeof(OpAlt::tab) / sizeof(OpAlt::Slot) == kOpMaxK + 1, "one entry per system and the alternate's");
std::string op_kernel_name(int K, const OpPlan& pl, int ek = 0);
std::string team_kernel_name(int K, const OpPlan& pl, int ek = 0);
int team_occupancy(const OpPlan& pl, int K, int ek = 0);
hipError_t atax(const Shard& s, const OpPlan& pl, int K, const OpArgs& a, hipStream_t st, const Timing& tm = Timing{},
                const int* gate = nullptr);
hipError_t atax_team(const Shard& s, const OpPlan& pl, int K, const OpArgs& a, hipStream_t st, const Timing& tm,
                     const int* gate);
hipError_t atax_team_plain(const Shard& s, const OpPlan& pl, const OpArgs& a, hipStream_t st, const Timing& tm,
                           const int* gate);
bool team_plain_plan(int64_t N, int64_t M, int cus, const OpPlan& main, OpPlan* out);
hipError_t op_reduce(const OpPlan& pl, int K, int64_t N, int64_t ld, const double* part, Ptrs out, double div,
                     hipStream_t st, const int* gate = nullptr, int k0 = 0);

hipError_t marker_stats(const Shard& s, double nonas, double alpha_scale, double* mave, double* msig,
                        hipStream_t st);

hipError_t gen_markers(uint64_t seed, int kind, int64_t N, int64_t ld, int64_t S, int64_t M, void* X, int ek,
                       hipStream_t st);
struct QuantRec {
    unsigned long long rejected;
    unsigned long long first;
    unsigned long long clamped;
    unsigned long long max_err;
};
hipError_t convert_cols(const void* src, int src_ek, int64_t lds, const int32_t* rows, int64_t n, int64_t ncols,
                        void* dst, int dst_ek, int64_t ldd, int64_t nfile, int64_t col0, QuantRec* rec,
                        hipStream_t st);
struct NaRec {
    unsigned long long missing;
    unsigned long long first;
    unsigned long long markers;
    unsigned long long masked;
};
enum { kNaFatal = 1, kNaMean = 2 };
hipError_t na_ingest_cols(const void* src, int src_ek, int64_t lds, const int32_t* rows, int64_t n, int64_t ncols,
                          void* dst, int dst_ek, int64_t ldd, int64_t nfile, int64_t col0, int mode, double max_frac,
                          int64_t* cnt, NaRec* nrec, QuantRec* qrec, hipStream_t st);
constexpr int kAdjMaxR = 65;
hipError_t adjust_cols(const double* src, int64_t n, int64_t ncols, const double* Q, int R, void* dst, int dst_ek,
                       int64_t ldd, uint8_t* flags, unsigned long long* absorbed, hipStream_t st);
hipError_t gen_beta(uint64_t seed, double lam, int64_t S, int64_t M, double* beta, const RedOut& ro, hipStream_t st);
hipError_t scale_vec(int64_t n, double* v, double a, hipStream_t st);
hipError_t add_noise(uint64_t seed, int64_t N, double sd, double* y, hipStream_t st);
// ... 214 lines not shown
constexpr unsigned long long kCgPackPre = 1ull << 31;
struct CgMirror {
    unsigned long long seq;
    int any;
    int iters[kMaxRhs];
};
constexpr int kCgMirrorSlots = 2;
hipError_t cg_start(const CgState& init, CgState* dst, hipStream_t st);
hipError_t cg_start_from(const CgState& init, const double* sums, CgState* dst, hipStream_t st,
                         const double* gam2dev = nullptr);
hipError_t prelude_cg_init(int K, int64_t M, const Prelude& p, const CgVecs& c, double diag, const RedOut& ro,
                           const CgState* start, CgState* dst, hipStream_t st);
struct CgDecide {
    int on = 0, it = 0;
    int pack = 0;
    int mask = 0xf;
    CgMirror* mirror = nullptr;
    unsigned long long* flag = nullptr;
    unsigned long long seq = 0;
};
hipError_t cg_update(int K, int64_t M, const CgVecs& c, double diag, CgState* cs, const double* dp_dev,
                     const double* pp_dev, int fuse, const RedOut& ro, const CgDecide& dc, hipStream_t st);
hipError_t cg_decide(CgState* cs, const double* red, int it, CgMirror* mirror, unsigned long long* flag,
                     unsigned long long seq, hipStream_t st, int mask = 0xf, int pack = 0);
struct PreCompose {
    const double* T1;
    const double* U1;
    const double* ab;
    const double* p;
    double* d;
    double* S;
    double* AD;
    double diag, tau, gam2;
};
hipError_t pre_compose(int64_t M, int64_t N, const PreCompose& a, const RedOut& ro, hipStream_t st);

}
```

### vampomi_amd/csrc/pcg.cpp

```cpp
#include <cstddef>
#include <string>

#include "ctx.h"

template <class T>
static T* field(vk::CgState* cs, size_t off) {
    return reinterpret_cast<T*>(reinterpret_cast<char*>(cs) + off);
}

struct CgOutcome {
    int any = 0;
    bool pre = false;
    int iters[vk::kMaxRhs] = {};
};

static constexpr int kCgPackWord = 2;

static vampomi_status read_packed(vampomi_ctx* c, int step, unsigned long long seq, CgOutcome* o) {
    const int word = kCgPackWord + (step & 1);
    STCHK(wait_flag(c, seq << 32, word));
    STCHK(op_check_err(c));
    const unsigned long long w = __atomic_load_n(c->h_flag + word, __ATOMIC_ACQUIRE);
    if ((w >> 32) != (seq & 0xffffffffULL))
        return fail(VAMPOMI_ERR_STATE, "CG step " + std::to_string(step) + ": decision word holds sequence " +
                                           std::to_string(w >> 32) + ", expected " + std::to_string(seq));
    o->any = (int)((w >> 30) & 1);
    o->pre = o->pre || (w & vk::kCgPackPre) != 0;
    o->iters[0] = (int)(w & 0x7fff);
    o->iters[1] = (int)((w >> 15) & 0x7fff);
    return VAMPOMI_OK;
}
static vampomi_status read_mirror(vampomi_ctx* c, int step, unsigned long long seq, CgOutcome* o) {
    STCHK(wait_flag(c, seq));
    STCHK(op_check_err(c));
    const vk::CgMirror* m = c->h_cgm + (step & 1);
    if (__atomic_load_n(&m->seq, __ATOMIC_ACQUIRE) != seq)
        return fail(VAMPOMI_ERR_STATE, "CG step " + std::to_string(step) + ": decision slot holds sequence " +
                                           std::to_string(m->seq) + ", expected " + std::to_string(seq));
    o->any = m->any;
    for (int k = 0; k < vk::kMaxRhs; ++k) o->iters[k] = m->iters[k];
    return VAMPOMI_OK;
}

template <class Solve>
static vampomi_status cg_loop(vampomi_ctx* c, int max_iter, bool packed, Solve& solve, CgOutcome* last) {
    unsigned long long prev = 0, cur = 0;
    STCHK(solve.enqueue(0, &prev));
    for (int i = 1;; ++i) {
        const size_t mark = c->pending.size();
        const vampomi_stats before = c->stats;
        if (i < max_iter)
            STCHK(solve.enqueue(i, &cur));
        else
            STCHK(solve.settle());
        c->stats.host_syncs++;
        STCHK(packed ? read_packed(c, i - 1, prev, last) : read_mirror(c, i - 1, prev, last));
        if (!last->any || i >= max_iter) {
            if (i < max_iter) drop_launches(c, mark, before);
            break;
        }
        prev = cur;
    }
    return VAMPOMI_OK;
}

struct Pcg {
    vampomi_ctx* c;
    const std::vector<CgSystem*>& sys;
    const PcgArgs& a;
    int K;
    double diag;
    bool rec;
    bool op1 = false;
    bool head = false;
    bool pre_ok = false;
    bool pre2 = false;
    const double* xnext() const { return a.hs ? a.hs->xnext : nullptr; }
    const int* gate() const { return field<int>(c->cgs, offsetof(vk::CgState, any)); }
    const double* beta() const { return field<double>(c->cgs, offsetof(vk::CgState, beta)); }
    vk::RedOut red(int slot, const int* g) const {
        return vk::RedOut{c->red_part, c->scal + slot, c->ticket, nullptr, 0, g};
    }
};

static vampomi_status copy_nvec(vampomi_ctx* c, double* dst, const double* src) {
    HIPCHK(hipMemcpyAsync(dst, src, (size_t)c->N * 8, hipMemcpyDeviceToDevice, c->st));
    return VAMPOMI_OK;
}

struct Product {
    const double* x;
    double* out;
};
static vampomi_status ax_products(vampomi_ctx* c, int n, const Product* pr, double* buf) {
    if (n == 0) return VAMPOMI_OK;
    const double* px[vk::kMaxRhs];
    for (int j = 0; j < n; ++j) px[j] = pr[j].x;
    STCHK(ax_dev(c, n, px, buf));
    for (int j = 0; j < n; ++j)
        if (pr[j].out != buf + (int64_t)j * c->ld) STCHK(copy_nvec(c, pr[j].out, buf + (int64_t)j * c->ld));
    return VAMPOMI_OK;
}
static vampomi_status extra_alone(const Pcg& s) {
    Product pr[2];
    int n = 0;
    if (s.a.extra_x) pr[n++] = {s.a.extra_x, s.a.ex_out};
    if (s.xnext()) pr[n++] = {s.xnext(), s.a.hs->axnext};
    return ax_products(s.c, n, pr, s.a.nscratch);
}
// ... 43 lines not shown
    if (a.pm != PreMode::normal && !a.pre) return fail(VAMPOMI_ERR_ARG, "pcg: a start queued ahead is the prelude's");
    if (a.pm != PreMode::normal && (a.pm == PreMode::ahead) != (a.pre->dev.scal != nullptr))
        return fail(VAMPOMI_ERR_ARG, "pcg: a start queued ahead needs the prelude and its device scalars");
    if (a.max_iter <= 0) return VAMPOMI_OK;
    for (int k = 0; a.onepass && K <= vk::kOpMaxK && a.ar0 && k < K; ++k)
        if (a.ar0[k] && sys[k]->mu0_nonzero) return fail(VAMPOMI_ERR_ARG, "pcg: A r0 given for a nonzero start");
    for (const CgSystem* y : sys)
        if (rec && !y->S) return fail(VAMPOMI_ERR_ARG, "pcg: W needs an S scratch vector for every system");
    return VAMPOMI_OK;
}

static vampomi_status pcg_start(Pcg& s, bool* go) {
    vampomi_ctx* c = s.c;
    const PcgArgs& a = s.a;
    const HeadStart* hs = a.hs;
    const int K = s.K;
    *go = false;
    {
        const double* vv[vk::kMaxRhs];
        double* dd[vk::kMaxRhs];
        int n = 0;
        for (CgSystem* y : s.sys) {
            if (y->mu0_nonzero && !y->atx0) vv[n] = y->mu, dd[n++] = y->d;
            if (y->mu0_nonzero && a.ref_passes) *a.ref_passes += 2;
        }
        if (n > 0) STCHK(lmmse_dev(c, n, vv, dd, a.tau, a.gam2, a.nscratch));
    }
    if (a.onepass && K <= vk::kOpMaxK && c->have_X) STCHK(op_prepare(c));
    s.op1 = a.onepass && K <= vk::kOpMaxK && c->have_X && c->op_ok;
    s.head = hs && hs->abern && c->hs_ok && c->op_ok && a.max_iter > 0;
    s.pre_ok = hs && s.op1 && !c->use_comm && c->opp.T >= 1 && hs->T1 && hs->U1 && hs->pre_done && a.max_iter > 0 &&
               a.max_iter < vk::kCgPackMaxIter;
    s.pre2 = s.head && s.pre_ok && hs->pre_have;
    vk::CgVecs cv = fill_vecs(s, false);
    for (int k = 0; k < K; ++k) {
        const CgSystem* y = s.sys[k];
        cv.atx0[k] = y->mu0_nonzero ? y->atx0 : nullptr;
        cv.d[k] = (y->mu0_nonzero && !y->atx0) ? y->d : nullptr;
    }
    vk::CgState s0{};
    s0.K = K;
    s0.gam2 = a.gam2;
    s0.tol = a.tol;
    s0.maxit = a.max_iter;
    s0.off[0] = s.head ? (s.pre2 ? 2 : 1) : 0;
    s0.any = a.max_iter > 0 ? 1 : 0;
    for (int k = 0; k < K; ++k) {
        s0.active[k] = 1;
        s0.onsager[k] = s.sys[k]->onsager ? 1 : 0;
        s.sys[k]->iters = 0;
    }
    if (a.init) {
        std::vector<double> rzvv(2 * K);
        vk::RedOut ro{};
        STCHK(a.init->sink(2 * K, true, rzvv.data(), &ro));
        HIPCHK(vk::cg_init(K, c->M, cv, s.diag, ro, c->st));
        STCHK(a.init->flush());
        for (int k = 0; k < K; ++k) {
            s0.rz[k] = rzvv[2 * k];
            s0.vv[k] = rzvv[2 * k + 1];
        }
        if (a.max_iter <= 0) return extra_alone(s);
        HIPCHK(vk::cg_start(s0, c->cgs, c->st));
    } else if (a.pm != PreMode::queued) {
        const vk::RedOut ro = s.red(SL_CGI, nullptr);
        const bool own_start = a.pre && !c->use_comm;
        if (a.pre)
            HIPCHK(vk::prelude_cg_init(K, c->M, *a.pre, cv, s.diag, ro, own_start ? &s0 : nullptr, c->cgs, c->st));
        else
            HIPCHK(vk::cg_init(K, c->M, cv, s.diag, ro, c->st));
        if (!own_start) {
            STCHK(allreduce_dev(c, c->scal + SL_CGI, (size_t)(2 * K)));
            if (a.max_iter > 0)
                HIPCHK(vk::cg_start_from(s0, c->scal + SL_CGI, c->cgs, c->st,
                                         a.pm == PreMode::ahead ? a.pre->dev.scal + 1 : nullptr));
        }
        if (a.pm == PreMode::ahead) return VAMPOMI_OK;
    }
    if (a.max_iter <= 0) return extra_alone(s);
    *go = true;
    return VAMPOMI_OK;
}

struct OnePassSolve : Pcg {
    HeadStart* const hs;
    double* const AR;
    double* const Q;
    const double* const AD;
    vk::CgVecs cu;
    const bool fold;
    int cur = 0;
    vk::OpFold pend;
    const bool packed;
    bool offer = false;
    unsigned long long token = 0;

    explicit OnePassSolve(const Pcg& s)
        : Pcg(s), hs(a.hs), AR(c->op_nvec), Q(AR + (int64_t)vk::kMaxRhs * c->ld),
          AD(AR + (int64_t)2 * vk::kMaxRhs * c->ld), cu(fill_vecs(s, true)),
          fold(c->use_comm && c->cg_fold && c->opp.T >= 1 && (!head || c->opp_hs.T >= 1)),
          packed(K <= 2 && a.max_iter < vk::kCgPackMaxIter) {
        cu.nA = c->N;
        for (int k = 0; k < K; ++k) {
            cu.Q[k] = Q + (int64_t)k * c->ld;
            cu.AR[k] = head && k == 0 ? hs->abern : AR + (int64_t)k * c->ld;
            cu.AD[k] = AD + (int64_t)k * c->ld;
        }
        if (!c->use_comm) {
            cu.adpart = c->op_part;
            cu.adld = c->ld;
            cu.adslots = c->opp.nslots;
        }
        cu.addiv = c->sqrtN;
    }
    vk::CgState* state(int i) const { return c->cgs + i; }
    vk::OpArgs op_args() const {
        vk::OpArgs o{};
        o.beta = beta();
        o.diag = diag;
        o.tau = a.tau;
        o.gam2 = a.gam2;
        return o;
    }
    void op_system(vk::OpArgs& o, int k) const {
        o.ar.p[k] = cu.AR[k];
        o.qo.p[k] = cu.Q[k];
        o.p.p[k] = sys[k]->p;
        o.z.p[k] = sys[k]->z;
        o.d.p[k] = sys[k]->d;
        o.sraw.p[k] = rec ? sys[k]->S : nullptr;
    }

    vampomi_status first_products() {
        Product pr[vk::kMaxRhs];
        int n = 0;
        bool given = false;
        for (int k = 0; k < K; ++k) {
            if (a.ar0 && a.ar0[k]) {
                given = true;
                STCHK(copy_nvec(c, AR + (int64_t)k * c->ld, a.ar0[k]));
            } else {
                pr[n++] = {sys[k]->r, AR + (int64_t)k * c->ld};
            }
        }
        if (a.extra_x) pr[n++] = {a.extra_x, a.ex_out};
        if (xnext()) pr[n++] = {xnext(), hs->axnext};
        return ax_products(c, n, pr, given ? a.nscratch : AR);
    }

    vampomi_status compose_step() {
        vk::PreCompose pc{};
        pc.T1 = hs->T1;
        pc.U1 = hs->U1;
        pc.ab = cu.AR[0];
        pc.p = sys[0]->p;
        pc.d = sys[0]->d;
        pc.S = rec ? sys[0]->S : nullptr;
        pc.AD = const_cast<double*>(cu.AD[0]);
        pc.diag = diag;
        pc.tau = a.tau;
        pc.gam2 = a.gam2;
        HIPCHK(vk::pre_compose(c->M, c->N, pc, red(SL_DP, gate()), c->st));
        vk::CgVecs cp = cu;
        cp.adpart = nullptr;
        cp.addiv = 0.0;
        vk::CgDecide dc{};
        dc.on = 1;
        dc.it = -2;
        dc.mask = 1;
        HIPCHK(vk::cg_update(1, c->M, cp, diag, c->cgs, c->scal + SL_DP, nullptr, 0, red(SL_CG, gate()), dc,
                             c->st));
        hs->pre_used = true;
        return VAMPOMI_OK;
    }

    vampomi_status head_step() {
        vk::OpArgs o = op_args();
        op_system(o, 0);
        o.fuse = pre2 ? 1 : 0;
        const double* xn = xnext();
        const double* px[vk::kOpPlain] = {sys[1]->r, a.extra_x, xn ? xn : a.extra_x};
        double* out[vk::kOpPlain] = {cu.AR[1], a.ex_out, xn ? hs->axnext : a.nscratch};
        STCHK(op_dev_plain(c, o, px, out, gate()));
        vk::CgVecs ch = cu;
        if (!c->use_comm) ch.adslots = (int)c->opp_hs.nslots;
        else ch.addiv = 0.0;
        const double* dp = c->use_comm ? AD + (int64_t)(1 + vk::kOpPlain) * c->ld : c->scal + SL_DP;
        vk::CgDecide dc{};
        dc.on = !c->use_comm;
        dc.it = -1;
        dc.mask = 1;
        HIPCHK(vk::cg_update(1, c->M, ch, diag, c->cgs, dp, nullptr, pre2 ? 1 : 0, red(SL_CG, gate()), dc,
                             c->st));
        if (c->use_comm) {
            STCHK(allreduce_dev(c, c->scal + SL_CG, 3));
            if (fold) {
                pend.on = 1;
                pend.it = -1;
                pend.mask = 1;
            } else {
                HIPCHK(vk::cg_decide(c->cgs, c->scal + SL_CG, -1, nullptr, nullptr, 0, c->st, 1));
            }
        }
        hs->used = true;
        return VAMPOMI_OK;
    }

    vampomi_status enqueue(int i, unsigned long long* seq) {
        const int fuse = i > 0 ? (1 << K) - 1 : head ? 1 : 0;
        vk::OpArgs o = op_args();
        for (int k = 0; k < K; ++k) op_system(o, k);
        if (offer) {
            o.alt.cs = c->cgs;
            o.alt.done = hs->pre_done;
            o.alt.token = token;
            o.alt.ar = hs->axnext;
            o.alt.p = hs->xnext;
            o.alt.d = hs->T1;
        }
        o.fuse = fuse;
        const int* g = gate();
        vk::CgState* cs = c->cgs;
        if (fold) {
            o.beta = nullptr;
            if (pend.on) {
                o.fold = pend;
                o.fold.src = state(cur);
                o.fold.dst = state(cur ^ 1);
                o.fold.red = c->scal + SL_CG;
                cur ^= 1;
                pend.on = 0;
            }
            cs = state(cur);
            g = field<int>(cs, offsetof(vk::CgState, any));
            if (!o.fold.on) o.beta = field<double>(cs, offsetof(vk::CgState, beta));
        }
        STCHK(op_dev(c, K, o, g, c->use_comm, false));
        const double* dp = c->use_comm ? AD + (int64_t)K * c->ld : c->scal + SL_DP;
        *seq = ++c->sync_seq;
        unsigned long long* flag = packed ? c->d_flag + kCgPackWord + (i & 1) : c->d_flag;
        vk::CgMirror* mirror = packed ? nullptr : c->d_cgm;
        vk::CgDecide dc{};
        if (!c->use_comm) {
            dc.on = 1;
            dc.it = i;
            dc.mirror = mirror;
            dc.flag = flag;
            dc.seq = *seq;
            dc.pack = packed ? 1 : 0;
        }
        HIPCHK(vk::cg_update(K, c->M, cu, diag, cs, dp, nullptr, fuse, red(SL_CG, g), dc, c->st));
        if (c->use_comm) {
            STCHK(allreduce_dev(c, c->scal + SL_CG, (size_t)(3 * K)));
            if (fold) {
                pend.on = 1;
                pend.it = i;
                pend.mask = 0xf;
                pend.pack = packed ? 1 : 0;
                pend.mirror = mirror;
                pend.flag = flag;
                pend.seq = *seq;
            } else {
                HIPCHK(vk::cg_decide(c->cgs, c->scal + SL_CG, i, mirror, flag, *seq, c->st, 0xf, packed ? 1 : 0));
            }
        }
        return VAMPOMI_OK;
    }

    vampomi_status settle() {
        if (!pend.on) return VAMPOMI_OK;
        HIPCHK(vk::cg_decide(state(cur), c->scal + SL_CG, pend.it, pend.mirror, pend.flag, pend.seq, c->st, pend.mask,
                             pend.pack));
        pend.on = 0;
        return VAMPOMI_OK;
    }

    vampomi_status finish(const CgOutcome& last) {
        STCHK(op_check_err(c));
        store_iters(*this, last);
        if (offer) hs->pre_made = last.pre;
        return VAMPOMI_OK;
    }

    vampomi_status run() {
        if (!head) STCHK(first_products());
        if (pre2) STCHK(compose_step());
        if (head) STCHK(head_step());
        offer = pre_ok && packed && hs->pre_offer && hs->xnext && hs->axnext && !fold;
        if (offer) {
            token = ++c->pre_seq;
            cu.pre_u1 = hs->U1;
            cu.pre_done = hs->pre_done;
            cu.pre_token = token;
        }
        CgOutcome last;
        STCHK(cg_loop(c, a.max_iter, packed, *this, &last));
        return finish(last);
    }
};

struct TwoPassSolve : Pcg {
    vk::CgVecs cu;
    double* dd[vk::kMaxRhs];
    double* ss[vk::kMaxRhs];
    const bool split_dp;

    explicit TwoPassSolve(const Pcg& s)
        : Pcg(s), cu(fill_vecs(s, true)), split_dp(c->use_comm && K < vk::kMaxRhs && !c->dp_separate) {
        for (int k = 0; k < K; ++k) {
            dd[k] = sys[k]->d;
            ss[k] = sys[k]->S;
            cu.AS[k] = a.nscratch + (int64_t)k * c->ld;
            if (sys[k]->AW) cu.nA = c->N;
        }
    }

    vampomi_status enqueue(int i, unsigned long long* seq) {
        const bool fuse = i > 0;
        vk::AxFuse fu{};
        fu.gate = gate();
        if (fuse) {
            for (int k = 0; k < K; ++k) fu.z.p[k] = cu.z[k];
            fu.beta = beta();
        }
        const double* px[vk::kMaxRhs];
        for (int k = 0; k < K; ++k) px[k] = cu.p[k];
        const bool ex = i == 0 && a.extra_x;
        if (ex) px[K] = a.extra_x;
        const int KA = ex ? K + 1 : K;
// ... 18 lines not shown
                      rec ? ss : nullptr));
        *seq = ++c->sync_seq;
        vk::CgDecide dc{};
        if (!c->use_comm) {
            dc.on = 1;
            dc.it = i;
            dc.mirror = c->d_cgm;
            dc.flag = c->d_flag;
            dc.seq = *seq;
        }
        HIPCHK(vk::cg_update(K, c->M, cu, diag, c->cgs, c->scal + SL_DP, pp_dev, fuse ? (1 << K) - 1 : 0,
                             red(SL_CG, gate()), dc, c->st));
        if (c->use_comm) {
            STCHK(allreduce_dev(c, c->scal + SL_CG, (size_t)(3 * K)));
            HIPCHK(vk::cg_decide(c->cgs, c->scal + SL_CG, i, c->d_cgm, c->d_flag, *seq, c->st));
        }
        return VAMPOMI_OK;
    }
    vampomi_status settle() { return VAMPOMI_OK; }

    vampomi_status run() {
        if (xnext()) {
            const Product pr{xnext(), a.hs->axnext};
            STCHK(ax_products(c, 1, &pr, a.nscratch));
        }
        CgOutcome last;
        STCHK(cg_loop(c, a.max_iter, false, *this, &last));
        store_iters(*this, last);
        return VAMPOMI_OK;
    }
};

vampomi_status pcg_run(vampomi_ctx* c, const std::vector<CgSystem*>& sys, const PcgArgs& args) {
    if (args.hs) args.hs->used = args.hs->pre_made = args.hs->pre_used = false;
    STCHK(pcg_check(c, sys, args));
    bool rec = false;
    for (const CgSystem* y : sys) rec = rec || y->W;
    const double diag = args.tau * (double)(c->N - 1) / (double)c->N + args.gam2;
    Pcg s{c, sys, args, (int)sys.size(), diag, rec};
    bool go = false;
    STCHK(pcg_start(s, &go));
    if (!go) return VAMPOMI_OK;
    return s.op1 ? OnePassSolve(s).run() : TwoPassSolve(s).run();
}
```

### vampomi_amd/csrc/pcg.hip

```cpp
#include "kernels.h"
#include "kdev.h"

#include <algorithm>
#include <cstdlib>

namespace vk {

__device__ __forceinline__ void cg_start_at(const CgVecs& c, int k, int64_t i, double vi, double atx0, double mu,
                                            double d, double tau, double gam2, double diag, double& rz, double& vv) {
    double r;
    if (c.atx0[k]) {
        double dv = atx0;
        dv *= tau;
        dv += gam2 * mu;
        r = vi - dv;
    } else {
        r = c.d[k] ? vi - d : vi - 0.0;
    }
    const double z = r / diag;
    c.r[k][i] = r;
    c.z[k][i] = z;
    c.p[k][i] = z;
    rz += r * z;
    vv += vi * vi;
// ... 350 lines not shown
        case 2: launch_cgu<2>(wide, mb + nb, st, M, c, diag, cs, dp_dev, pp_dev, fuse, ro, dc, mb); break;
        case 3: launch_cgu<3>(wide, mb + nb, st, M, c, diag, cs, dp_dev, pp_dev, fuse, ro, dc, mb); break;
        case 4: launch_cgu<4>(wide, mb + nb, st, M, c, diag, cs, dp_dev, pp_dev, fuse, ro, dc, mb); break;
        default: return hipErrorInvalidValue;
    }
    return hipGetLastError();
}

hipError_t cg_decide(CgState* cs, const double* red, int it, CgMirror* mirror, unsigned long long* flag,
                     unsigned long long seq, hipStream_t st, int mask, int pack) {
    hipLaunchKernelGGL(cg_decide_kernel, dim3(1), dim3(64), 0, st, cs, red, it, mirror, flag, seq, mask, pack);
    return hipGetLastError();
}

__global__ __launch_bounds__(kBlock) void pre_compose_kernel(int64_t M, int64_t N, PreCompose a, RedOut ro) {
    if (ro.gate && !*ro.gate) return;
    __shared__ double lds[4];
    double acc[1] = {0.0};
    const int64_t stride = (int64_t)gridDim.x * kBlock;
    for (int64_t i = (int64_t)blockIdx.x * kBlock + threadIdx.x; i < M; i += stride) {
        const double t = a.T1[i] / a.diag;
        const double p = a.p[i];
        double d = t * a.tau;
        d += a.gam2 * p;
        a.d[i] = d;
        if (a.S) a.S[i] = t;
        acc[0] += d * p;
    }
    for (int64_t j = (int64_t)blockIdx.x * kBlock + threadIdx.x; j < N; j += stride) {
        double u = a.tau * a.U1[j];
        u += a.gam2 * a.ab[j];
        a.AD[j] = u / a.diag;
    }
    block_put_sums<1>(acc, 1, ro, (int64_t)blockIdx.x);
    red_finish(ro, 1, lds);
}

hipError_t pre_compose(int64_t M, int64_t N, const PreCompose& a, const RedOut& ro, hipStream_t st) {
    hipLaunchKernelGGL(pre_compose_kernel, dim3(red_blocks(M)), dim3(kBlock), 0, st, M, N, a, ro);
    return hipGetLastError();
}

}
```

### vampomi_amd/csrc/run.h

```cpp
#pragma once
#include <string>
#include <vector>

#include "ctx.h"
#include "writer.h"

struct Mixture {
    int L = 0;
    double probs[VAMPOMI_MAX_L] = {};
    double vars[VAMPOMI_MAX_L] = {};
};

inline double smax(double a, double b) { return (a < b) ? b : a; }
inline double smin(double a, double b) { return (b < a) ? b : a; }

struct VampRun {
    vampomi_params prm{};
    vampomi_result* res = nullptr;
    bool probit = false;
    bool write = false;
    bool fuse = true;
    bool recur = false;
    bool arec = false;
    bool onepass = false;
    int z1n_slot = 2;
    int bern_it = 0;
    int abern_it = 0;
    int em_head = 0, z_head = 0;
    double zh_bsum = 0, zh_cnt[4] = {}, zh_xc[3] = {};
    int hs_it = 0;
    std::string out_dir, out_name, p_params, p_metrics, p_prior;
    int it = 0;
    bool stopped = false;
    bool io_err = false;
    std::string io_msg;
    IterWriter* writer = nullptr;
    Mixture mix, mix_next;
    bool have_next = false;
    double gam1 = 0, gam2 = 0, gamw = 0;
    double alpha1 = 0, alpha2 = 0, eta1 = 0, eta2 = 0, alpha1_next = 0;
    double metrics[12] = {}, params[8] = {};
    double e1m[3] = {}, e1n[2] = {}, e1s[3] = {}, e2m[3] = {}, e2n[2] = {}, e2s[3] = {};
    double tn = 0, tc = 0, nm[2] = {}, sum_d = 0, a2 = 0;
    double *r1 = nullptr, *x1 = nullptr, *x1p = nullptr, *x1n = nullptr, *x1d = nullptr, *r2 = nullptr;
    double *x2 = nullptr, *bern = nullptr, *invQ = nullptr, *v = nullptr, *atxy = nullptr, *ts = nullptr;
    double *tmpM = nullptr, *atx0 = nullptr;
    double* cgw[10] = {};
    double *z1buf = nullptr, *nb3 = nullptr , *nsc = nullptr;
    double* ax2 = nullptr;
    double* abern = nullptr;
    double* bern_next = nullptr;
    double* pre_t1 = nullptr;
    double* pre_u1 = nullptr;
    int pre_it = 0;
    double* mixw = nullptr;
    double* mixh = nullptr;
    double* mixh_dev = nullptr;
    bool mix_pending = false;
    Mixture mix_expect;
    int pre_ahead = 0;
    bool pre_ahead_on = true;
    const double* z1 = nullptr;
    int64_t passes_ref = 0;
    double tau1 = 0, tau2 = 0, beta1 = 0, beta2 = 0;
    double* p1 = nullptr;
    double* p2 = nullptr;
    double* z1h = nullptr;
    double* x1s = nullptr;
    double* x1sn = nullptr;
    double* x2s = nullptr;
    double* m_cov = nullptr;
    double* prior_row = nullptr;
    double ph_solve_s = 0, ph_step_s = 0;

    ~VampRun();
};

struct EmParams {
    int EM_max_iter;
    double EM_err_thr;
    int learn_vars;
    double merge_vars_thr;
    int verbosity;
};
EmParams em_params(const VampRun& R);
vampomi_status update_prior(vampomi_ctx* c, const EmParams& P, Mixture& m, double gam1, const double* r1);
vampomi_status update_prior(vampomi_ctx* c, const VampRun& R, Mixture& m, double gam1, const double* r1);
// ... 30 lines not shown
```

### vampomi_amd/csrc/vamp.cpp

```cpp
#include <algorithm>
#include <chrono>
#include <cmath>
#include <cstdio>
#include <cstring>

#include "ctx.h"
#include "hostio.h"
#include "run.h"

VampRun::~VampRun() {
    if (writer) writer->drain(nullptr);
    for (double** p : {&r1, &x1, &x1p, &x1n, &x1d, &r2, &x2, &bern, &invQ, &v, &atxy, &ts, &tmpM, &atx0, &z1buf,
                       &nb3, &nsc, &ax2, &p1, &p2, &z1h, &x1s, &x1sn, &x2s, &abern, &bern_next, &pre_t1, &pre_u1, &m_cov})
        dev_free(*p);
    for (auto& p : cgw) dev_free(p);
    dev_free(mixw);
    if (mixh) (void)hipHostFree(mixh);
}

vampomi_ctx::vampomi_ctx() = default;

vampomi_ctx::~vampomi_ctx() {
    run.reset();
    writer.reset();
    release_ctx_resources(this);
}

vampomi_status em_begin(vampomi_ctx* c, const EmParams& P, const Mixture& m, double gam1, const double* r1,
                        DotBatch& b, EmState& s, const R1From* r1from, const vk::EmUpd* upd) {
    s.emit = 0;
    s.lambda = 1 - m.probs[0];
    for (int j = 0; j < m.L; ++j) s.omegas[j] = m.probs[j];
    for (int j = 1; j < m.L; ++j) s.omegas[j] /= s.lambda;
    if (P.EM_max_iter < 1) return VAMPOMI_OK;
    return em_queue(c, m, gam1, r1, b, s, r1from, upd);
}

vampomi_status em_queue(vampomi_ctx* c, const Mixture& m, double gam1, const double* r1, DotBatch& b,
                        EmState& s, const R1From* r1from, const vk::EmUpd* upd) {
    const int L = m.L;
    double max_sigma = m.vars[0];
    for (int j = 1; j < L; ++j) max_sigma = smax(max_sigma, m.vars[j]);
    vk::EmArgs a{};
    for (int j = 0; j < L; ++j) {
        a.omegas[j] = s.omegas[j];
        a.vars[j] = m.vars[j];
// ... 364 lines not shown
    sx.r = R.cgw[0];
    sx.z = R.cgw[1];
    sx.p = R.cgw[2];
    sx.d = R.cgw[3];
    so.v = R.bern;
    so.mu = R.invQ;
    so.onsager = true;
    so.r = R.cgw[4];
    so.z = R.cgw[5];
    so.p = R.cgw[6];
    so.d = R.cgw[7];
    L.rec = R.recur && R.fuse && (it == 1 || sx.atx0);
    if (L.rec) {
        sx.W = R.atx0;
        sx.S = R.cgw[8];
        so.W = R.tmpM;
        so.S = R.cgw[9];
    }
    L.arec = R.arec && L.rec;
    if (L.arec) sx.AW = R.ax2;
    if (R.fuse && L.arec && R.onepass) STCHK(headstart_available(c, &L.hs_av));
    if (L.hs_av) {
        L.hs.abern = R.hs_it == it ? R.abern + (it & 1) * ld : nullptr;
        if (it < R.prm.max_iter) {
            L.hs.xnext = R.bern_next;
            L.hs.axnext = R.abern + ((it + 1) & 1) * ld;
        }
        if (prestep_on(c)) {
            L.hs.T1 = R.pre_t1;
            L.hs.U1 = R.pre_u1;
            L.hs.pre_done = reinterpret_cast<unsigned long long*>(R.pre_u1 + ld);
            L.hs.pre_have = L.hs.abern && R.pre_it == it;
            L.hs.pre_offer = L.hs.xnext != nullptr;
        }
    }
    vk::Prelude& pr = L.pr;
    pr.eta1 = R.eta1;
    pr.gam1 = R.gam1;
    pr.gam2 = R.gam2;
    pr.gamw = R.gamw;
    pr.x1 = x1;
    pr.r1 = R.r1;
    pr.atxy = R.atxy;
    pr.r2 = R.r2;
    pr.v = R.v;
    pr.seed = R.prm.seed;
    pr.it = it;
    pr.S = c->S;
    pr.sqrtMt = std::sqrt((double)c->Mt);
    pr.bern = R.bern;
    pr.bern_next = L.hs.xnext ? R.bern_next : nullptr;
    pr.zero[0] = R.invQ;
    pr.zero[1] = L.rec ? R.tmpM : nullptr;
    L.pre_in_cg = R.fuse && (L.hs_av || L.arec);
    return VAMPOMI_OK;
}

static vampomi_status check_device_values(vampomi_ctx* c, VampRun& R, int it) {
    STCHK(check_device_mix(R));
    if (R.pre_ahead != it) return VAMPOMI_OK;
    R.pre_ahead = 0;
    const double diag = R.gamw * (double)(c->N - 1) / (double)c->N + R.gam2;
    const double want[4] = {R.eta1, R.gam2, R.gamw, diag};
    if (std::memcmp(want, R.mixh + vk::kMixWords, sizeof want) != 0)
        return fail(VAMPOMI_ERR_STATE, "vamp: the prelude queued ahead formed other scalars than the host");
    return VAMPOMI_OK;
// ... 50 lines not shown
        a.extra_x = x1;
        a.ex_out = R.z1buf;
        a.pre = &L.pr;
    }
    if (L.hs_av) {
        a.hs = &L.hs;
        a.pm = pm;
    }
    return a;
}

static vampomi_status lmmse_solves(vampomi_ctx* c, VampRun& R, int it, LmmseSetup& L, DotBatch& e1) {
    const int64_t M = c->M, ld = c->ld;
    vampomi_result* res = R.res;
    CgSystem& sx = L.sx;
    CgSystem& so = L.so;
    HeadStart& hs = L.hs;
    R.passes_ref += 1;
    if (it == 1) {
        HIPCHK(hipMemsetAsync(R.x2, 0, (size_t)std::max<int64_t>(M, 1) * 8, c->st));
        if (L.rec) HIPCHK(hipMemsetAsync(R.atx0, 0, (size_t)std::max<int64_t>(M, 1) * 8, c->st));
        if (L.arec) HIPCHK(hipMemsetAsync(R.ax2, 0, (size_t)ld * 8, c->st));
    }
    const PreMode pm = R.pre_ahead == it ? PreMode::queued : PreMode::normal;
    if (pm == PreMode::queued && !(L.pre_in_cg && R.fuse && L.hs_av))
        return fail(VAMPOMI_ERR_STATE, "vamp: the start queued ahead does not match this iteration's schedule");
    if (!L.pre_in_cg) HIPCHK(vk::prelude(M, L.pr, c->st));
    const auto t_solve = std::chrono::steady_clock::now();
    PcgArgs pargs = pcg_args(R, L, R.x1, pm);
    if (R.fuse && L.hs_av) {
        STCHK(pcg_run(c, {&so, &sx}, pargs));
        R.hs_it = hs.xnext ? it + 1 : 0;
        R.pre_it = hs.pre_made ? it + 1 : 0;
        c->pre_made_n += hs.pre_made ? 1 : 0;
        c->pre_used_n += hs.pre_used ? 1 : 0;
    } else if (R.fuse) {
        if (!L.arec) pargs.init = &e1;
        STCHK(pcg_run(c, {&sx, &so}, pargs));
        R.hs_it = R.pre_it = 0;
    } else {
        R.pre_it = 0;
        PcgArgs first = pargs;
        first.init = &e1;
        STCHK(pcg_run(c, {&sx}, first));
        STCHK(pcg_run(c, {&so}, pargs));
    }
    R.ph_solve_s = std::chrono::duration<double>(std::chrono::steady_clock::now() - t_solve).count();
    STCHK(check_device_values(c, R, it));
    if (res && res->cg_iters) res->cg_iters[it - 1] = sx.iters;
    if (res && res->ons_iters) res->ons_iters[it - 1] = so.iters;
    return VAMPOMI_OK;
}

struct TailPlan {
    bool next = false;
    bool em_next = false;
    bool r1_in_em = false;
    bool chain = false, mr = false;
    bool devem = false;
    bool ahead = false;
    LmmseSetup A;
    vk::PreOut po;
};

static vampomi_status tail_plan(vampomi_ctx* c, VampRun& R, int it, const LmmseSetup& L, TailPlan& t) {
    t.next = R.fuse && it < R.prm.max_iter;
    t.em_next = t.next && it + 1 > R.prm.learn_prior_delay;
    t.r1_in_em = t.next && L.arec && t.em_next && R.prm.EM_max_iter >= 1;
// ... 387 lines not shown
```

Baseline: 183.3.

## Precompute two next-iteration CG steps via a third system in the team kernel

Extends the head-start prestep so the fused A/A^T team kernel carries a third right-hand side during the first two CG iterations, precomputing two Krylov products for the next VAMP iteration instead of one. A new compose2 kernel combines the saved products with the CG scalars, which should let the next iteration skip an extra pass over the matrix. It adds K=3 team kernel instantiations with narrower lane groups, extra buffers and reductions, and more complex state bookkeeping. The extra system also raises per-pass work and may lower occupancy in the kernels that carry it.

```diff
diff --git a/include/vampomi.h b/include/vampomi.h
--- a/include/vampomi.h
+++ b/include/vampomi.h
@@ -227,6 +227,8 @@
 vampomi_status vampomi_dev_op_plan(int64_t N, int64_t M, int cus, int variant, int K, int* T, int* S, int* TR,
                                    int* grid, int64_t* nslots, char* name, int cap);
 vampomi_status vampomi_dev_op_lds(int64_t N, int64_t M, int cus, int variant, int K, int64_t* out);
+vampomi_status vampomi_dev_op3_plan(int64_t N, int64_t M, int cus, int variant, int* T, int* S, int* TR, int* grid,
+                                    int* cfg, int64_t* nslots, char* name, int cap, int64_t* lds);
 vampomi_status vampomi_dev_op_timestamps(vampomi_ctx* ctx, unsigned long long* out, int cap, int* n);
 vampomi_status vampomi_dev_mem_plan(int64_t N, int64_t Mt, int nranks, int rank, int cus, int probit, int writer,
                                     int64_t* bytes);
@@ -235,6 +237,9 @@
 vampomi_status vampomi_dev_op_apply(vampomi_ctx* ctx, int K, const double* ar, const double* qo, const double* p,
                                     const double* z, const double* beta, double diag, double tau, double gam2,
                                     double* d, double* ad, double* dp);
+vampomi_status vampomi_dev_op_apply3(vampomi_ctx* ctx, const double* ar, const double* qo, const double* p,
+                                     const double* z, const double* beta, double diag, double tau, double gam2,
+                                     const double* ar3, const double* p3, double* d, double* ad, double* dp);
 
 #ifdef __cplusplus
 }
diff --git a/vampomi_amd/__init__.py b/vampomi_amd/__init__.py
--- a/vampomi_amd/__init__.py
+++ b/vampomi_amd/__init__.py
@@ -472,6 +472,28 @@
                                              _dp(d), _dp(ad), _dp(dp)))
         return d[:, : self.M], ad, dp
 
+    def op_apply3(self, ar, p, diag: float, tau: float, gam2: float, ar3, p3, z=None, qo=None, beta=None):
+        ar = np.ascontiguousarray(ar, dtype=np.float64)
+        p = np.ascontiguousarray(p, dtype=np.float64)
+        ar3 = np.ascontiguousarray(ar3, dtype=np.float64)
+        p3 = np.ascontiguousarray(p3, dtype=np.float64)
+        if ar.shape != (2, self.N) or p.shape != (2, self.M) or ar3.shape != (self.N,) or p3.shape != (self.M,):
+            raise ValueError("ar must be 2 x N, p 2 x M, ar3 N and p3 M")
+        fz = z is not None
+        if fz:
+            z = np.ascontiguousarray(z, dtype=np.float64)
+            qo = np.ascontiguousarray(qo, dtype=np.float64)
+            beta = np.ascontiguousarray(beta, dtype=np.float64)
+            if z.shape != (2, self.M) or qo.shape != (2, self.N) or beta.shape != (2,):
+                raise ValueError("z must be 2 x M, qo 2 x N and beta 2")
+        d = np.zeros((3, max(self.M, 1)))
+        ad = np.zeros((3, self.N))
+        dp = np.zeros(2)
+        check(self._lib.vampomi_dev_op_apply3(self.ctx, _dp(ar), _dp(qo) if fz else None, _dp(p),
+                                              _dp(z) if fz else None, _dp(beta) if fz else None, diag, tau, gam2,
+                                              _dp(ar3), _dp(p3), _dp(d), _dp(ad), _dp(dp)))
+        return d[:, : self.M], ad, dp
+
     def read_ceiling(self, reps: int = 9) -> dict:
         us, nb, var = C.c_double(), C.c_double(), C.c_int()
         check(self._lib.vampomi_dev_read_ceiling(self.ctx, int(reps), C.byref(us), C.byref(nb), C.byref(var)))
diff --git a/vampomi_amd/_lib.py b/vampomi_amd/_lib.py
--- a/vampomi_amd/_lib.py
+++ b/vampomi_amd/_lib.py
@@ -177,6 +177,10 @@
     "vampomi_dev_op_lds": (C.c_int, [C.c_int64, C.c_int64, C.c_int, C.c_int, C.c_int, _P]),
     "vampomi_dev_op_apply": (C.c_int, [_P, C.c_int, _P, _P, _P, _P, _P, C.c_double, C.c_double, C.c_double, _P, _P,
                                        _P]),
+    "vampomi_dev_op3_plan": (C.c_int, [C.c_int64, C.c_int64, C.c_int, C.c_int, _P, _P, _P, _P, _P, _P, C.c_char_p,
+                                       C.c_int, _P]),
+    "vampomi_dev_op_apply3": (C.c_int, [_P, _P, _P, _P, _P, _P, C.c_double, C.c_double, C.c_double, _P, _P, _P, _P,
+                                        _P]),
     "vampomi_dev_op_timestamps": (C.c_int, [_P, _P, C.c_int, C.POINTER(C.c_int)]),
     "vampomi_all_ok": (C.c_int, [_P, C.c_int, C.POINTER(C.c_int)]),
     "vampomi_comm_abort": (C.c_int, [_P]),
diff --git a/vampomi_amd/csrc/atax_team.hip b/vampomi_amd/csrc/atax_team.hip
--- a/vampomi_amd/csrc/atax_team.hip
+++ b/vampomi_amd/csrc/atax_team.hip
@@ -199,7 +199,7 @@
     TmSlots<K> s;
 #pragma unroll
     for (int k = 0; k < K; ++k) {
-        int idx = k == alt ? kOpMaxK : k;
+        int idx = k == alt || k >= kOpMaxK ? kOpMaxK : k;
         asm volatile("" : "+s"(idx));
         const OpAlt::Slot& t = a.alt.tab[idx];
         s.ar[k] = t.ar;
@@ -243,6 +243,10 @@
     }
     const double* beta = a.fold.on ? s_beta : a.beta;
     static_assert(K + KP <= kMaxRhs, "partial slots per team");
+    static_assert(K <= kOpSys && (K <= kOpMaxK || (COMM && KP == 0)), "a third system: team plans only");
+    constexpr int KD = K < kOpMaxK ? K : kOpMaxK;
+    constexpr int KG = K > kOpMaxK ? K : kOpMaxK;
+    constexpr int GW = K > 2 ? 16 : 32;
     int fuse = a.fuse, alt = -1;
     if constexpr (KP == 0) {
         if (a.alt.cs && !a.fold.on) alt = cg_pre_slot(a.alt.cs->active, K, *a.alt.done == a.alt.token);
@@ -272,7 +276,7 @@
     const int64_t mb = ilv ? team : (int64_t)team * M / nteams;
     const int n = (int)(ilv ? (M - team + nteams - 1) / nteams : (int64_t)(team + 1) * M / nteams - mb);
     const int64_t nmax = (M + nteams - 1) / nteams;
-    const int64_t gwords = (M + gridDim.x) * kOpMaxK * T * 2;
+    const int64_t gwords = (M + gridDim.x) * KG * T * 2;
     const int64_t r0 = (int64_t)member * TR;
     const int nrows = (int)(N - r0 < TR ? N - r0 : TR);
     constexpr bool QFULL = tm_qfull(K, S, COMM, E);
@@ -290,8 +294,8 @@
         const int nq = K * T;
         unsigned long long* xg = a.xg + (int64_t)team * nmax * nq * 2;
         unsigned long long* dummy = a.xg + gwords + (int64_t)blockIdx.x * 2 * K;
-        const bool qv = (lane >> 5) < K && (lane & 31) < T;
-        const int ql2 = qv ? 2 * ((lane >> 5) * T + (lane & 31)) : 0;
+        const bool qv = (lane / GW) < K && (lane % GW) < T;
+        const int ql2 = qv ? 2 * ((lane / GW) * T + (lane % GW)) : 0;
         const int nq2 = 2 * nq;
         const int csi = (int)cs;
         const unsigned tag = a.tag;
@@ -299,13 +303,13 @@
 #pragma unroll
         for (int k = 0; k < K; ++k) {
             if (lane == 1 + k) scp = sl.p[k];
-            if (lane == 1 + K + k && ((fuse >> k) & 1)) scp = a.z.p[k];
+            if (k < kOpMaxK && lane == 1 + K + k && ((fuse >> k) & 1)) scp = a.z.p[k];
         }
         scp += mb;
         double bk[K], dpacc[K];
 #pragma unroll
         for (int k = 0; k < K; ++k) {
-            bk[k] = ((fuse >> k) & 1) ? beta[k] : 0.0;
+            bk[k] = k < kOpMaxK && ((fuse >> k) & 1) ? beta[k] : 0.0;
             dpacc[k] = 0.0;
         }
         v4u pl[RING];
@@ -315,7 +319,7 @@
         if (n > 0) {
             bool l2 = false;
             {
-                unsigned long long* hdr = a.xg + gwords + (int64_t)gridDim.x * 2 * kOpMaxK + (int64_t)team * T;
+                unsigned long long* hdr = a.xg + gwords + (int64_t)gridDim.x * 2 * KG + (int64_t)team * T;
                 unsigned xcc;
                 asm volatile("s_getreg_b32 %0, hwreg(HW_REG_XCC_ID)" : "=s"(xcc));
                 xcc &= 0xf;
@@ -375,7 +379,7 @@
                         if (dbg & 512) {
                             for (int o = T >> 1; o > 0; o >>= 1) v += __shfl_xor(v, o, 64);
                         } else if (!(dbg & 256)) {
-                            v = group_sum<32>(v);
+                            v = group_sum<GW>(v);
                         }
                         const double scv = __builtin_bit_cast(double, ((unsigned long long)sc.y << 32) | sc.x);
                         const double sg = readlane_d(scv, 0);
@@ -384,10 +388,10 @@
                         double tsc[K], dval[K], pdir[K];
 #pragma unroll
                         for (int k = 0; k < K; ++k) {
-                            double t = sg * readlane_d(v, 32 * k);
+                            double t = sg * readlane_d(v, GW * k);
                             t *= a.scale;
                             double p = readlane_d(scv, 1 + k);
-                            if ((fuse >> k) & 1) p = readlane_d(scv, 1 + K + k) + bk[k] * p;
+                            if (k < kOpMaxK && ((fuse >> k) & 1)) p = readlane_d(scv, 1 + K + k) + bk[k] * p;
                             double val = t * sl.tau[k];
                             val += sl.gam2[k] * p;
                             tsc[k] = t;
@@ -417,7 +421,7 @@
                         const v4u gr = {(unsigned)u, tag, (unsigned)(u >> 32), tag};
                         unsigned long long* dst =
                             tm_chk(real ? xg + ((int64_t)m * nq2 + (lane * T + member) * 2) : dummy + 2 * lane, a.xg,
-                                   a.xg + gwords + (int64_t)gridDim.x * 2 * kOpMaxK, 512, a.err);
+                                   a.xg + gwords + (int64_t)gridDim.x * 2 * KG, 512, a.err);
                         if (l2)
                             tm_publish_l2(dst, gr);
                         else
@@ -435,7 +439,7 @@
         }
         if (lane == 0) {
 #pragma unroll
-            for (int k = 0; k < K; ++k) red_put(a.ro, (int64_t)blockIdx.x * K + k, dpacc[k]);
+            for (int k = 0; k < KD; ++k) red_put(a.ro, (int64_t)blockIdx.x * KD + k, dpacc[k]);
         }
         asm volatile("s_waitcnt vmcnt(0)" ::: "memory");
         __syncthreads();
@@ -455,7 +459,7 @@
                 if (jl + h < nrows) {
                     const int64_t j = r0 + jl + h;
                     q = sl.ar[k][j] / sl.diag[k];
-                    if ((fuse >> k) & 1) q = q + beta[k] * a.qo.p[k][j];
+                    if (k < kOpMaxK && ((fuse >> k) & 1)) q = q + beta[k] * a.qo.p[k][j];
                 }
                 q_lds[k * QS + jl + h] = q;
             }
@@ -463,13 +467,13 @@
     }
     double bk[K];
 #pragma unroll
-    for (int k = 0; k < K; ++k) bk[k] = ((fuse >> k) & 1) ? beta[k] : 0.0;
+    for (int k = 0; k < K; ++k) bk[k] = k < kOpMaxK && ((fuse >> k) & 1) ? beta[k] : 0.0;
     const double* pkp = mave;
     if (lane == 1) pkp = msig;
 #pragma unroll
     for (int k = 0; k < K; ++k) {
         if (lane == 2 + k) pkp = sl.p[k];
-        if (lane == 2 + K + k && ((fuse >> k) & 1)) pkp = a.z.p[k];
+        if (k < kOpMaxK && lane == 2 + K + k && ((fuse >> k) & 1)) pkp = a.z.p[k];
     }
 #pragma unroll
     for (int k = 0; k < KP; ++k)
@@ -582,9 +586,9 @@
                 }
             }
         }
-        if (K == 2) {
+        if (K >= 2) {
             double r0, r1;
-            swap32(v[0], v[K - 1], r0, r1);
+            swap32(v[0], v[K >= 2 ? 1 : 0], r0, r1);
             double keep = r0 + r1;
             if (dbg & 512) {
                 for (int o = 16; o > 0; o >>= 1) keep += __shfl_xor(keep, o, 64);
@@ -592,6 +596,10 @@
                 keep = group_sum<32>(keep);
             }
             if ((lane & 31) == 0) s_part[(par * CW + wave) * K + (lane >> 5)] = keep;
+            if constexpr (K == 3) {
+                if (!(dbg & 4)) v[K - 1] = group_sum<64>(v[K - 1]);
+                if (lane == 0) s_part[(par * CW + wave) * K + K - 1] = v[K - 1];
+            }
         } else {
             if (!(dbg & 4)) v[0] = group_sum<64>(v[0]);
             if (lane == 0) s_part[(par * CW + wave) * K] = v[0];
@@ -611,7 +619,7 @@
                 double t = sg * tot[k];
                 t *= a.scale;
                 double p = readlane_d(pk[slot], 2 + k);
-                if ((fuse >> k) & 1) p = readlane_d(pk[slot], 2 + K + k) + bk[k] * p;
+                if (k < kOpMaxK && ((fuse >> k) & 1)) p = readlane_d(pk[slot], 2 + K + k) + bk[k] * p;
                 double val = t * sl.tau[k];
                 val += sl.gam2[k] * p;
                 if (own) {
@@ -696,9 +704,9 @@
         __syncthreads();
     } else if (threadIdx.x == 0) {
 #pragma unroll
-        for (int k = 0; k < K; ++k) red_put(a.ro, (int64_t)blockIdx.x * K + k, dpacc[k]);
-    }
-    if (wave == 0) ticket_sum_blocks<K>(a.ro);
+        for (int k = 0; k < KD; ++k) red_put(a.ro, (int64_t)blockIdx.x * KD + k, dpacc[k]);
+    }
+    if (wave == 0) ticket_sum_blocks<KD>(a.ro);
 #if TM_TS
     if (a.ts && threadIdx.x == 0) {
         unsigned xcc, hw;
@@ -932,8 +940,32 @@
     return true;
 }
 
+static constexpr int tm_sys3_maxS(int cfg) { return cfg == 2 ? 3 : cfg == 4 ? 4 : 0; }
+static constexpr int kTmSys3MaxT = 16;
+
+bool team_sys3_ok(const OpPlan& pl) {
+    if (pl.cfg < 0 || pl.cfg >= kTmNCfg || pl.T < 2 || pl.T > kTmSys3MaxT || pl.S < 1 || pl.S > tm_sys3_maxS(pl.cfg))
+        return false;
+    const TmCfg& c = kTmCfg[pl.cfg];
+    return tm_lds(kOpSys, pl.S, c.comm, c.E, pl.TR).words * 8 <= kTmLdsMaxBytes;
+}
+
+bool team_sys3_plan(int64_t N, int64_t M, int cus, const OpPlan& main, OpPlan* out) {
+    if (main.T < 2) return false;
+    for (int T = main.T; T <= kTmSys3MaxT; T *= 2) {
+        for (int cfg : {2, 4}) {
+            OpPlan p{};
+            if (!team_plan(N, M, cus, T, cfg, &p) || !team_sys3_ok(p)) continue;
+            *out = p;
+            return true;
+        }
+    }
+    return false;
+}
+
 bool team_lds_layout(const OpPlan& pl, int64_t N, int K, int64_t out[6]) {
-    if (pl.T < 1 || pl.cfg < 0 || pl.cfg >= kTmNCfg || K < 1 || K > kOpMaxK || N < 1) return false;
+    if (pl.T < 1 || pl.cfg < 0 || pl.cfg >= kTmNCfg || K < 1 || N < 1) return false;
+    if (K > kOpMaxK && !(K == kOpSys && team_sys3_ok(pl))) return false;
     const TmCfg& c = kTmCfg[pl.cfg];
     const TmLds l = tm_lds(K, pl.S, c.comm, c.E, std::min<int64_t>(pl.TR, N));
     out[0] = kTmLdsHead;
@@ -995,7 +1027,7 @@
 template <int K, int C, int S, bool PL>
 static hipError_t launch_tm_if(const Shard& s, const OpPlan& pl, const OpArgs& a, hipStream_t st, const Timing& tm,
                                const int* gate, int* occ) {
-    if constexpr (S <= (PL ? tm_plain_maxS(C) : kTmCfg[C].maxS))
+    if constexpr (S <= (PL ? tm_plain_maxS(C) : K == kOpSys ? tm_sys3_maxS(C) : kTmCfg[C].maxS))
         return launch_tm<K, S, C, PL>(s, pl, a, st, tm, gate, occ);
     return hipErrorInvalidValue;
 }
@@ -1039,6 +1071,13 @@
             default: return hipErrorInvalidValue;
         }
     }
+    if constexpr (K == kOpSys) {
+        switch (pl.cfg) {
+            case 2: return launch_tm_s<K, 2, false>(pl.S, s, pl, a, st, tm, gate, occ);
+            case 4: return launch_tm_s<K, 4, false>(pl.S, s, pl, a, st, tm, gate, occ);
+            default: return hipErrorInvalidValue;
+        }
+    }
     switch (pl.cfg) {
         case 0: return launch_tm_s<K, 0, false>(pl.S, s, pl, a, st, tm, gate, occ);
         case 1: return launch_tm_s<K, 1, false>(pl.S, s, pl, a, st, tm, gate, occ);
@@ -1060,6 +1099,11 @@
     switch (K) {
         case 1: e = launch_tm_c<1>(s, pl, a, st, tm, gate); break;
         case 2: e = launch_tm_c<2>(s, pl, a, st, tm, gate); break;
+        case kOpSys:
+            if (!team_sys3_ok(pl) || a.fold.on || a.alt.cs || (a.fuse >> kOpMaxK) || !a.alt.ar || !a.alt.p || !a.alt.d)
+                return hipErrorInvalidValue;
+            e = launch_tm_c<kOpSys>(s, pl, a, st, tm, gate);
+            break;
         default: break;
     }
     if (e != hipSuccess) return e;
@@ -1180,6 +1224,7 @@
     switch (K) {
         case 1: e = launch_tm_c<1>(s, pl, a, nullptr, Timing{}, nullptr, &occ); break;
         case 2: e = launch_tm_c<2>(s, pl, a, nullptr, Timing{}, nullptr, &occ); break;
+        case kOpSys: e = team_sys3_ok(pl) ? launch_tm_c<kOpSys>(s, pl, a, nullptr, Timing{}, nullptr, &occ) : e; break;
         case 1 + kTmPlain: e = launch_tm_c<1, true>(s, pl, a, nullptr, Timing{}, nullptr, &occ); break;
         default: break;
     }
diff --git a/vampomi_amd/csrc/ctx.h b/vampomi_amd/csrc/ctx.h
--- a/vampomi_amd/csrc/ctx.h
+++ b/vampomi_amd/csrc/ctx.h
@@ -145,6 +145,8 @@
     bool hs_ok = false;
     bool hs_on = true;
     bool hs_on_req = true;
+    vk::OpPlan opp3{};
+    bool sys3_ok = false;
     int pre_mode = 2;
     unsigned long long pre_seq = 0;
     int64_t pre_made_n = 0, pre_used_n = 0;
@@ -273,6 +275,13 @@
     bool pre_offer = false;
     bool pre_made = false;
     bool pre_used = false;
+    bool pre3 = false;
+    double* T2 = nullptr;
+    double* U2 = nullptr;
+    double* rz_save = nullptr;
+    int n_have = 0;
+    int n_made = 0;
+    int n_used = 0;
 };
 enum class PreMode { normal, ahead, queued };
 struct PcgArgs {
@@ -296,6 +305,9 @@
 vampomi_status headstart_available(vampomi_ctx* c, bool* yes);
 constexpr int64_t kPreMinBytes = (int64_t)256 << 20;
 bool prestep_on(const vampomi_ctx* c);
+int prestep_mode(const vampomi_ctx* c);
+constexpr bool kPreAutoThird = true;
+bool prestep_wants3(const vampomi_ctx* c);
 unsigned* op_err_dev(vampomi_ctx* c);
 vampomi_status op_check_err(vampomi_ctx* c);
 vampomi_status op_dev(vampomi_ctx* c, int K, const vk::OpArgs& a, const int* gate, bool reduce = true,
diff --git a/vampomi_amd/csrc/engine.cpp b/vampomi_amd/csrc/engine.cpp
--- a/vampomi_amd/csrc/engine.cpp
+++ b/vampomi_amd/csrc/engine.cpp
@@ -674,8 +674,8 @@
                              (size_t)(Mx / 8 + 1) * vk::kMaxRhs, (size_t)4096});
 }
 
-static size_t op_xg_words_for(int64_t Mx, const vk::OpPlan& p) {
-    return (size_t)(Mx + p.grid) * vk::kOpMaxK * (size_t)p.T * 2 + (size_t)p.grid * (2 * vk::kOpMaxK + 1);
+static size_t op_xg_words_for(int64_t Mx, const vk::OpPlan& p, int K = vk::kOpMaxK) {
+    return (size_t)(Mx + p.grid) * K * (size_t)p.T * 2 + (size_t)p.grid * (2 * K + 1);
 }
 
 static vampomi_status op_plan_local(vampomi_ctx* c) {
@@ -695,8 +695,11 @@
     }
     bool hs_ok = op_ok && vk::team_plain_plan(c->N, M, c->cus, c->opp, &c->opp_hs);
     if (hs_ok && (int64_t)vk::team_occupancy(c->opp_hs, 1 + vk::kOpPlain, c->ek()) * c->cus < c->opp_hs.grid) hs_ok = false;
+    bool sys3_ok = op_ok && vk::team_sys3_plan(c->N, M, c->cus, c->opp, &c->opp3);
+    if (sys3_ok && (int64_t)vk::team_occupancy(c->opp3, vk::kOpSys, c->ek()) * c->cus < c->opp3.grid) sys3_ok = false;
     c->op_ok_mine = op_ok;
     c->hs_ok_mine = hs_ok;
+    c->sys3_ok = sys3_ok;
     if (!c->op_ts && std::getenv("VAMPOMI_OP_TS") && std::atoi(std::getenv("VAMPOMI_OP_TS"))) {
         HIPCHK(hipMalloc((void**)&c->op_ts, (size_t)4 * 8 * std::max(c->cus, 1) * 2));
         HIPCHK(hipMemsetAsync(c->op_ts, 0, (size_t)4 * 8 * std::max(c->cus, 1) * 2, c->st));
@@ -706,7 +709,8 @@
         HIPCHK(hipMemsetAsync(c->op_nvec, 0, ((size_t)3 * vk::kMaxRhs * c->ld + 16) * 8, c->st));
     }
     if (op_ok) {
-        const int64_t slots = std::max<int64_t>(c->opp.nslots, hs_ok ? c->opp_hs.nslots : 0);
+        const int64_t slots =
+            std::max<int64_t>({c->opp.nslots, hs_ok ? c->opp_hs.nslots : 0, sys3_ok ? c->opp3.nslots : 0});
         if (slots > c->op_part_slots) {
             dev_free(c->op_part);
             STCHK(dev_alloc(&c->op_part, (size_t)slots * vk::kMaxRhs * c->ld));
@@ -715,6 +719,7 @@
         if (c->opp.T > 1 || (hs_ok && c->opp_hs.T > 1)) {
             size_t words = c->opp.T > 1 ? op_xg_words_for(M, c->opp) : 0;
             if (hs_ok && c->opp_hs.T > 1) words = std::max(words, op_xg_words_for(M, c->opp_hs));
+            if (sys3_ok) words = std::max(words, op_xg_words_for(M, c->opp3, vk::kOpSys));
             if (words > c->op_xg_words) {
                 if (c->op_xg) (void)hipFree(c->op_xg);
                 c->op_xg = nullptr;
@@ -845,13 +850,16 @@
 vampomi_status op_dev(vampomi_ctx* c, int K, const vk::OpArgs& a, const int* gate, bool reduce, bool divide) {
     if (!c->have_X) return fail(VAMPOMI_ERR_STATE, "A before the methylation data was loaded");
     STCHK(op_prepare(c));
-    if (!c->op_ok || K < 1 || K > vk::kOpMaxK)
-        return fail(VAMPOMI_ERR_ARG, "one-pass operator: K <= 2 and a plan for N = " + std::to_string(c->N));
+    if (!c->op_ok || K < 1 || K > vk::kOpSys)
+        return fail(VAMPOMI_ERR_ARG, "one-pass operator: K <= 3 and a plan for N = " + std::to_string(c->N));
+    if (K == vk::kOpSys && (!c->sys3_ok || c->use_comm))
+        return fail(VAMPOMI_ERR_ARG, "one-pass operator: no 3-system plan for N = " + std::to_string(c->N));
+    const vk::OpPlan& pl = K == vk::kOpSys ? c->opp3 : c->opp;
     double* ad = c->op_nvec + (int64_t)2 * vk::kMaxRhs * c->ld;
     vk::OpArgs x = a;
     x.part = c->op_part;
     x.scale = 1.0 / c->sqrtN;
-    if (c->opp.T > 1) {
+    if (pl.T > 1) {
         x.xg = c->op_xg;
         if (++c->op_tag == 0) ++c->op_tag;
         x.tag = c->op_tag;
@@ -863,13 +871,12 @@
     x.ro = vk::RedOut{c->red_part, c->use_comm ? ad + (int64_t)K * c->ld : c->scal + SL_DP, c->ticket, nullptr, 0,
                       gate};
     TimedLaunch t = launch_stat(c, 3, K, pass_bytes(c, K), 2.0 * pass_flops(c, K));
-    STCHK(team_launch(c, c->opp.T,
-                      [&] { return vk::atax(c->shard(), c->opp, K, x, c->st, vk::Timing{t.a, t.b}, gate); }));
+    STCHK(team_launch(c, pl.T, [&] { return vk::atax(c->shard(), pl, K, x, c->st, vk::Timing{t.a, t.b}, gate); }));
     c->stats.a_passes_exec++;
     vk::Ptrs os{};
     for (int k = 0; k < K; ++k) os.p[k] = ad + (int64_t)k * c->ld;
     if (!c->use_comm) {
-        if (reduce) HIPCHK(vk::op_reduce(c->opp, K, c->N, c->ld, c->op_part, os, c->sqrtN, c->st, gate));
+        if (reduce) HIPCHK(vk::op_reduce(pl, K, c->N, c->ld, c->op_part, os, c->sqrtN, c->st, gate));
     } else {
         HIPCHK(vk::op_reduce(c->opp, K, c->N, c->ld, c->op_part, os, 0.0, c->st, gate));
         STCHK(allreduce_dev(c, ad, (size_t)K * c->ld + K));
@@ -1079,7 +1086,7 @@
     if (const char* hv = std::getenv("VAMPOMI_HEADSTART")) c->hs_on = c->hs_on_req = std::atoi(hv) != 0;
     if (const char* pv = std::getenv("VAMPOMI_PRESTEP")) {
         const int v = std::atoi(pv);
-        if (v >= 0 && v <= 2) c->pre_mode = v;
+        if (v >= 0 && v <= 3) c->pre_mode = v;
     }
     const char* mode = std::getenv("VAMPOMI_COMM");
     if (c->use_comm && mode && std::strcmp(mode, "loopback") == 0) {
@@ -1561,7 +1568,7 @@
         c->hs_on_req = variant == 1;
         if (!c->use_comm) c->hs_on = c->hs_on_req;
     } else if (which == 7) {
-        if (variant < 0 || variant > 2) return fail(VAMPOMI_ERR_ARG, "pre-step: 0, 1 or 2");
+        if (variant < 0 || variant > 3) return fail(VAMPOMI_ERR_ARG, "pre-step: 0, 1, 2 or 3");
         c->pre_mode = variant;
     } else if (which == 6) {
         if (variant != 0 && variant != 1) return fail(VAMPOMI_ERR_ARG, "multi-rank tail: 0 or 1");
@@ -1576,7 +1583,15 @@
 
 bool prestep_on(const vampomi_ctx* c) {
     if (c->use_comm || c->nranks != 1 || !c->hs_ok || c->pre_mode == 0) return false;
-    return c->pre_mode == 1 || std::max<int64_t>(c->M, 1) * c->ld * c->esize() >= kPreMinBytes;
+    return c->pre_mode == 1 || c->pre_mode == 3 ||
+           std::max<int64_t>(c->M, 1) * c->ld * c->esize() >= kPreMinBytes;
+}
+
+bool prestep_wants3(const vampomi_ctx* c) { return c->pre_mode == 3 || (c->pre_mode == 2 && kPreAutoThird); }
+
+int prestep_mode(const vampomi_ctx* c) {
+    if (!prestep_on(c)) return 0;
+    return prestep_wants3(c) && c->sys3_ok ? 3 : 1;
 }
 
 extern "C" vampomi_status vampomi_dev_prestep_counts(const vampomi_ctx* c, int64_t* made, int64_t* used) {
@@ -1587,13 +1602,14 @@
 }
 
 extern "C" vampomi_status vampomi_dev_time_pass(vampomi_ctx* c, int which, int K, int reps, double* avg_ms) {
-    if (!c || !avg_ms || K < 1 || K > (which == 0 ? 4 : which == 1 ? 3 : which == 3 ? 2 : 1) || reps < 1)
+    if (!c || !avg_ms || K < 1 || K > (which == 0 ? 4 : which == 1 ? 3 : which == 3 ? 3 : 1) || reps < 1)
         return fail(VAMPOMI_ERR_ARG, "bad argument");
     if (!c->have_X) return fail(VAMPOMI_ERR_STATE, "no methylation data loaded");
     HIPCHK(hipSetDevice(c->device));
     if (which == 3) {
         STCHK(op_prepare(c));
         if (!c->op_ok_mine) return fail(VAMPOMI_ERR_ARG, "no one-pass operator plan for this N");
+        if (K == vk::kOpSys && !c->sys3_ok) return fail(VAMPOMI_ERR_ARG, "no 3-system operator plan for this N");
     }
     const int64_t Mx = std::max<int64_t>(c->M, 1);
     vk::CPtrs in{};
@@ -1612,27 +1628,33 @@
         else if (which == 1)
             HIPCHK(vk::atx(c->shard(), K, in, out, 1.0 / c->sqrtN, 0, 0.0, 0.0, vk::CPtrs{}, c->st, c->atx_variant));
         else if (which == 3) {
+            const vk::OpPlan& pl = K == vk::kOpSys ? c->opp3 : c->opp;
             vk::OpArgs x{};
-            for (int k = 0; k < K; ++k) {
+            for (int k = 0; k < K && k < vk::kOpMaxK; ++k) {
                 x.ar.p[k] = c->nbuf + k * c->ld;
                 x.p.p[k] = c->mbuf + k * Mx;
                 x.d.p[k] = c->mbuf + (2 + k) * Mx;
+            }
+            if (K == vk::kOpSys) {
+                x.alt.ar = c->nbuf + 2 * c->ld;
+                x.alt.p = c->mbuf + 4 * Mx;
+                x.alt.d = c->mbuf + 5 * Mx;
             }
             x.diag = 1.0;
             x.scale = 1.0 / c->sqrtN;
             x.tau = 1.0;
             x.part = c->op_part;
             x.ro = vk::RedOut{c->red_part, c->scal + SL_DP, c->ticket, nullptr, 0, nullptr};
-            if (c->opp.T > 1) {
+            if (pl.T > 1) {
                 x.xg = c->op_xg;
                 if (++c->op_tag == 0) ++c->op_tag;
                 x.tag = c->op_tag;
                 x.err = op_err_dev(c);
             }
             x.dbg = std::getenv("VAMPOMI_OP_DBG") ? std::atoi(std::getenv("VAMPOMI_OP_DBG")) : 0;
-            if (c->opp.T > 1) x.err = op_err_dev(c);
+            if (pl.T > 1) x.err = op_err_dev(c);
             x.ts = c->op_ts;
-            STCHK(team_launch(c, c->opp.T, [&] { return vk::atax(c->shard(), c->opp, K, x, c->st); }));
+            STCHK(team_launch(c, pl.T, [&] { return vk::atax(c->shard(), pl, K, x, c->st); }));
         }
         else
             HIPCHK(vk::loo_sums(c->shard(), c->nbuf, c->mbuf, c->sqrtN, c->mbuf + 3 * Mx, c->st, c->loo_variant));
@@ -1700,6 +1722,58 @@
     return op_check_err(c);
 }
 
+extern "C" vampomi_status vampomi_dev_op_apply3(vampomi_ctx* c, const double* ar, const double* qo, const double* p,
+                                                const double* z, const double* beta, double diag, double tau,
+                                                double gam2, const double* ar3, const double* p3, double* d,
+                                                double* ad, double* dp) {
+    constexpr int K = vk::kOpMaxK;
+    if (!c || !ar || !p || !ar3 || !p3 || !d || !ad || !dp || (z && (!qo || !beta)))
+        return fail(VAMPOMI_ERR_ARG, "bad argument");
+    if (c->use_comm) return fail(VAMPOMI_ERR_ARG, "vampomi_dev_op_apply3: one rank only");
+    HIPCHK(hipSetDevice(c->device));
+    STCHK(op_prepare(c));
+    if (!c->op_ok || !c->sys3_ok) return fail(VAMPOMI_ERR_ARG, "no 3-system operator plan for this N");
+    const int64_t Mx = std::max<int64_t>(c->M, 1);
+    double* AR = c->op_nvec;
+    double* Q = c->op_nvec + (int64_t)vk::kMaxRhs * c->ld;
+    vk::OpArgs a{};
+    for (int k = 0; k < K; ++k) {
+        STCHK(stage_in(c, ar + k * c->N, c->N, VAMPOMI_MEM_HOST, AR + k * c->ld));
+        STCHK(stage_in(c, p + k * c->M, c->M, VAMPOMI_MEM_HOST, c->mbuf + k * Mx));
+        a.ar.p[k] = AR + k * c->ld;
+        a.p.p[k] = c->mbuf + k * Mx;
+        a.d.p[k] = c->mbuf + (2 + k) * Mx;
+        if (z) {
+            STCHK(stage_in(c, qo + k * c->N, c->N, VAMPOMI_MEM_HOST, Q + k * c->ld));
+            STCHK(stage_in(c, z + k * c->M, c->M, VAMPOMI_MEM_HOST, c->mbuf + (4 + k) * Mx));
+            a.qo.p[k] = Q + k * c->ld;
+            a.z.p[k] = c->mbuf + (4 + k) * Mx;
+        }
+    }
+    STCHK(stage_in(c, ar3, c->N, VAMPOMI_MEM_HOST, AR + K * c->ld));
+    STCHK(stage_in(c, p3, c->M, VAMPOMI_MEM_HOST, c->mbuf + 6 * Mx));
+    a.alt.ar = AR + K * c->ld;
+    a.alt.p = c->mbuf + 6 * Mx;
+    a.alt.d = c->mbuf + 7 * Mx;
+    if (z) {
+        STCHK(stage_in(c, beta, K, VAMPOMI_MEM_HOST, c->nbuf));
+        a.beta = c->nbuf;
+        a.fuse = (1 << K) - 1;
+    }
+    a.diag = diag;
+    a.tau = tau;
+    a.gam2 = gam2;
+    STCHK(op_dev(c, vk::kOpSys, a, nullptr));
+    const double* AD = c->op_nvec + (int64_t)2 * vk::kMaxRhs * c->ld;
+    for (int k = 0; k < vk::kOpSys; ++k) {
+        STCHK(stage_out(c, k < K ? c->mbuf + (2 + k) * Mx : c->mbuf + 7 * Mx, c->M, VAMPOMI_MEM_HOST, d + k * c->M));
+        STCHK(stage_out(c, AD + k * c->ld, c->N, VAMPOMI_MEM_HOST, ad + k * c->N));
+    }
+    HIPCHK(hipMemcpyAsync(dp, c->scal + SL_DP, (size_t)K * 8, hipMemcpyDeviceToHost, c->st));
+    STCHK(sync_stream(c, c->st));
+    return op_check_err(c);
+}
+
 extern "C" vampomi_status vampomi_dev_op_timestamps(vampomi_ctx* c, unsigned long long* out, int cap, int* n) {
     if (!c || !out || !n) return fail(VAMPOMI_ERR_ARG, "null argument");
     if (!c->op_ts) return fail(VAMPOMI_ERR_STATE, "no timestamps (VAMPOMI_OP_TS=1 at the first operator use)");
@@ -1739,8 +1813,27 @@
 
 extern "C" vampomi_status vampomi_dev_op_lds(int64_t N, int64_t M, int cus, int variant, int K, int64_t* out) {
     vk::OpPlan p{};
-    if (!out || !vk::op_plan(N, std::max<int64_t>(M, 1), cus, variant, &p) || !vk::team_lds_layout(p, N, K, out))
+    if (!out || K > vk::kOpMaxK || !vk::op_plan(N, std::max<int64_t>(M, 1), cus, variant, &p) ||
+        !vk::team_lds_layout(p, N, K, out))
         return fail(VAMPOMI_ERR_ARG, "no team plan with that system count");
+    return VAMPOMI_OK;
+}
+
+extern "C" vampomi_status vampomi_dev_op3_plan(int64_t N, int64_t M, int cus, int variant, int* T, int* S, int* TR,
+                                               int* grid, int* cfg, int64_t* nslots, char* name, int cap,
+                                               int64_t* lds) {
+    vk::OpPlan main{}, p{};
+    const int64_t Mx = std::max<int64_t>(M, 1);
+    if (!vk::op_plan(N, Mx, cus, variant, &main) || !vk::team_sys3_plan(N, Mx, cus, main, &p))
+        return fail(VAMPOMI_ERR_ARG, "no 3-system operator plan");
+    if (lds && !vk::team_lds_layout(p, N, vk::kOpSys, lds)) return fail(VAMPOMI_ERR_ARG, "no 3-system operator plan");
+    if (T) *T = p.T;
+    if (S) *S = p.S;
+    if (TR) *TR = p.TR;
+    if (grid) *grid = p.grid;
+    if (cfg) *cfg = p.cfg;
+    if (nslots) *nslots = p.nslots;
+    if (name && cap > 0) std::snprintf(name, (size_t)cap, "%s", vk::team_kernel_name(vk::kOpSys, p).c_str());
     return VAMPOMI_OK;
 }
 
@@ -1769,16 +1862,27 @@
     vk::OpPlan op{}, hs{};
     if (vk::op_plan(N, Mx, cus, vk::kOpDefault, &op)) {
         const bool h = vk::team_plain_plan(N, Mx, cus, op, &hs);
+        vk::OpPlan s3{};
+        const bool h3 = vk::team_sys3_plan(N, Mx, cus, op, &s3);
         add((int64_t)3 * vk::kMaxRhs * ld + 16, 8);
-        add(std::max<int64_t>(op.nslots, h ? hs.nslots : 0) * vk::kMaxRhs * ld, 8);
+        add(std::max<int64_t>({op.nslots, h ? hs.nslots : 0, h3 ? s3.nslots : 0}) * vk::kMaxRhs * ld, 8);
         size_t w = op.T > 1 ? op_xg_words_for(Mx, op) : 0;
         if (h && hs.T > 1) w = std::max(w, op_xg_words_for(Mx, hs));
+        if (h3) w = std::max(w, op_xg_words_for(Mx, s3, vk::kOpSys));
         if (w) add((int64_t)w, 8);
     }
     for (int q = 0; q < 25; ++q) add(Mx, 8);
     add(ld, 8), add((int64_t)vk::kMaxRhs * ld, 8), add((int64_t)vk::kMaxRhs * ld, 8), add(ld, 8);
     add(2 * ld, 8);
     add(Mx, 8), add(ld + 2, 8);
+    {
+        vk::OpPlan s3{};
+        const bool auto3 = kPreAutoThird && nranks == 1 && !probit && vk::op_plan(N, Mx, cus, vk::kOpDefault, &op) &&
+                           vk::team_sys3_plan(N, Mx, cus, op, &s3) &&
+                           Mx * ld * (storage == VAMPOMI_STORE_F32 ? 4 : storage == VAMPOMI_STORE_U16 ? 2 : 8) >=
+                               kPreMinBytes;
+        if (auto3) add(Mx, 8), add(ld + 2, 8);
+    }
     if (probit) {
         for (int q = 0; q < 3; ++q) add(ld, 8);
         for (int q = 0; q < 3; ++q) add(Mx, 8);
@@ -1804,6 +1908,11 @@
         vk::OpPlan h{};
         if (!vk::team_plain_plan(c->N, std::max<int64_t>(c->M, 1), cus, p, &h)) return "(no head-start plan)";
         return vk::team_kernel_name(K, h, c->ek());
+    }
+    if (K == vk::kOpSys) {
+        vk::OpPlan t{};
+        if (!vk::team_sys3_plan(c->N, std::max<int64_t>(c->M, 1), cus, p, &t)) return "(no 3-system plan)";
+        return vk::team_kernel_name(K, t, c->ek());
     }
     return vk::op_kernel_name(K, p, c->ek());
 }
diff --git a/vampomi_amd/csrc/kernels.h b/vampomi_amd/csrc/kernels.h
--- a/vampomi_amd/csrc/kernels.h
+++ b/vampomi_amd/csrc/kernels.h
@@ -86,6 +86,7 @@
                const int* gate = nullptr, CPtrs zf = CPtrs{}, const double* beta = nullptr, Ptrs sraw = Ptrs{});
 
 constexpr int kOpMaxK = 2;
+constexpr int kOpSys = kOpMaxK + 1;
 constexpr int kOpPlain = 3;
 struct OpPlan {
     int grid;
@@ -157,6 +158,8 @@
 hipError_t atax_team_plain(const Shard& s, const OpPlan& pl, const OpArgs& a, hipStream_t st, const Timing& tm,
                            const int* gate);
 bool team_plain_plan(int64_t N, int64_t M, int cus, const OpPlan& main, OpPlan* out);
+bool team_sys3_plan(int64_t N, int64_t M, int cus, const OpPlan& main, OpPlan* out);
+bool team_sys3_ok(const OpPlan& pl);
 hipError_t op_reduce(const OpPlan& pl, int K, int64_t N, int64_t ld, const double* part, Ptrs out, double div,
                      hipStream_t st, const int* gate = nullptr, int k0 = 0);
 
@@ -437,7 +440,27 @@
     double* S;
     double* AD;
     double diag, tau, gam2;
+    const CgState* cs = nullptr;
+    double* rz_save = nullptr;
 };
 hipError_t pre_compose(int64_t M, int64_t N, const PreCompose& a, const RedOut& ro, hipStream_t st);
+struct PreCompose2 {
+    const double* T1;
+    const double* T2;
+    const double* U1;
+    const double* U2;
+    const double* ar;
+    const double* q;
+    const double* p;
+    const double* z;
+    double* d;
+    double* S;
+    double* AD;
+    double diag, tau, gam2;
+    const CgState* cs;
+    const double* rz_save;
+    const double* dp0;
+};
+hipError_t pre_compose2(int64_t M, int64_t N, const PreCompose2& a, const RedOut& ro, hipStream_t st);
 
 }
diff --git a/vampomi_amd/csrc/pcg.cpp b/vampomi_amd/csrc/pcg.cpp
--- a/vampomi_amd/csrc/pcg.cpp
+++ b/vampomi_amd/csrc/pcg.cpp
@@ -1,3 +1,4 @@
+#include <algorithm>
 #include <cstddef>
 #include <string>
 
@@ -43,7 +44,8 @@
 }
 
 template <class Solve>
-static vampomi_status cg_loop(vampomi_ctx* c, int max_iter, bool packed, Solve& solve, CgOutcome* last) {
+static vampomi_status cg_loop(vampomi_ctx* c, int max_iter, bool packed, Solve& solve, CgOutcome* last,
+                              int* nrun = nullptr) {
     unsigned long long prev = 0, cur = 0;
     STCHK(solve.enqueue(0, &prev));
     for (int i = 1;; ++i) {
@@ -57,6 +59,7 @@
         STCHK(packed ? read_packed(c, i - 1, prev, last) : read_mirror(c, i - 1, prev, last));
         if (!last->any || i >= max_iter) {
             if (i < max_iter) drop_launches(c, mark, before);
+            if (nrun) *nrun = i;
             break;
         }
         prev = cur;
@@ -75,6 +78,7 @@
     bool head = false;
     bool pre_ok = false;
     bool pre2 = false;
+    int J = 0;
     const double* xnext() const { return a.hs ? a.hs->xnext : nullptr; }
     const int* gate() const { return field<int>(c->cgs, offsetof(vk::CgState, any)); }
     const double* beta() const { return field<double>(c->cgs, offsetof(vk::CgState, beta)); }
@@ -184,6 +188,7 @@
     s.pre_ok = hs && s.op1 && !c->use_comm && c->opp.T >= 1 && hs->T1 && hs->U1 && hs->pre_done && a.max_iter > 0 &&
                a.max_iter < vk::kCgPackMaxIter;
     s.pre2 = s.head && s.pre_ok && hs->pre_have;
+    s.J = !s.pre2 ? 0 : hs->pre3 && hs->n_have >= 2 ? 2 : 1;
     vk::CgVecs cv = fill_vecs(s, false);
     for (int k = 0; k < K; ++k) {
         const CgSystem* y = s.sys[k];
@@ -195,7 +200,7 @@
     s0.gam2 = a.gam2;
     s0.tol = a.tol;
     s0.maxit = a.max_iter;
-    s0.off[0] = s.head ? (s.pre2 ? 2 : 1) : 0;
+    s0.off[0] = s.head ? 1 + s.J : 0;
     s0.any = a.max_iter > 0 ? 1 : 0;
     for (int k = 0; k < K; ++k) {
         s0.active[k] = 1;
@@ -246,6 +251,8 @@
     const bool packed;
     bool offer = false;
     unsigned long long token = 0;
+    bool offer3 = false;
+    int nrun = 0;
 
     explicit OnePassSolve(const Pcg& s)
         : Pcg(s), hs(a.hs), AR(c->op_nvec), Q(AR + (int64_t)vk::kMaxRhs * c->ld),
@@ -312,7 +319,45 @@
         pc.diag = diag;
         pc.tau = a.tau;
         pc.gam2 = a.gam2;
+        if (J == 2) {
+            pc.cs = c->cgs;
+            pc.rz_save = hs->rz_save;
+        }
         HIPCHK(vk::pre_compose(c->M, c->N, pc, red(SL_DP, gate()), c->st));
+        vk::CgVecs cp = cu;
+        cp.adpart = nullptr;
+        cp.addiv = 0.0;
+        vk::CgDecide dc{};
+        dc.on = 1;
+        dc.it = -1 - J;
+        dc.mask = 1;
+        HIPCHK(vk::cg_update(1, c->M, cp, diag, c->cgs, c->scal + SL_DP, nullptr, 0, red(SL_CG, gate()), dc,
+                             c->st));
+        hs->pre_used = true;
+        hs->n_used = J;
+        return VAMPOMI_OK;
+    }
+
+    vampomi_status compose_step2() {
+        vk::PreCompose2 pc{};
+        pc.T1 = hs->T1;
+        pc.T2 = hs->T2;
+        pc.U1 = hs->U1;
+        pc.U2 = hs->U2;
+        pc.ar = cu.AR[0];
+        pc.q = cu.Q[0];
+        pc.p = sys[0]->p;
+        pc.z = sys[0]->z;
+        pc.d = sys[0]->d;
+        pc.S = rec ? sys[0]->S : nullptr;
+        pc.AD = const_cast<double*>(cu.AD[0]);
+        pc.diag = diag;
+        pc.tau = a.tau;
+        pc.gam2 = a.gam2;
+        pc.cs = c->cgs;
+        pc.rz_save = hs->rz_save;
+        pc.dp0 = c->scal + SL_DP;
+        HIPCHK(vk::pre_compose2(c->M, c->N, pc, red(SL_DP, gate()), c->st));
         vk::CgVecs cp = cu;
         cp.adpart = nullptr;
         cp.addiv = 0.0;
@@ -320,9 +365,8 @@
         dc.on = 1;
         dc.it = -2;
         dc.mask = 1;
-        HIPCHK(vk::cg_update(1, c->M, cp, diag, c->cgs, c->scal + SL_DP, nullptr, 0, red(SL_CG, gate()), dc,
+        HIPCHK(vk::cg_update(1, c->M, cp, diag, c->cgs, c->scal + SL_DP, nullptr, 1, red(SL_CG, gate()), dc,
                              c->st));
-        hs->pre_used = true;
         return VAMPOMI_OK;
     }
 
@@ -362,6 +406,12 @@
         const int fuse = i > 0 ? (1 << K) - 1 : head ? 1 : 0;
         vk::OpArgs o = op_args();
         for (int k = 0; k < K; ++k) op_system(o, k);
+        const bool third = offer3 && i < 2;
+        if (third) {
+            o.alt.ar = i == 0 ? hs->axnext : hs->U1;
+            o.alt.p = i == 0 ? hs->xnext : hs->T1;
+            o.alt.d = i == 0 ? hs->T1 : hs->T2;
+        }
         if (offer) {
             o.alt.cs = c->cgs;
             o.alt.done = hs->pre_done;
@@ -387,7 +437,14 @@
             g = field<int>(cs, offsetof(vk::CgState, any));
             if (!o.fold.on) o.beta = field<double>(cs, offsetof(vk::CgState, beta));
         }
-        STCHK(op_dev(c, K, o, g, c->use_comm, false));
+        STCHK(op_dev(c, third ? vk::kOpSys : K, o, g, c->use_comm, false));
+        vk::CgVecs cv = cu;
+        if (third) {
+            vk::Ptrs us{};
+            us.p[0] = i == 0 ? hs->U1 : hs->U2;
+            HIPCHK(vk::op_reduce(c->opp3, 1, c->N, c->ld, c->op_part, us, c->sqrtN, c->st, g, vk::kOpMaxK));
+            cv.adslots = (int)c->opp3.nslots;
+        }
         const double* dp = c->use_comm ? AD + (int64_t)K * c->ld : c->scal + SL_DP;
         *seq = ++c->sync_seq;
         unsigned long long* flag = packed ? c->d_flag + kCgPackWord + (i & 1) : c->d_flag;
@@ -401,7 +458,7 @@
             dc.seq = *seq;
             dc.pack = packed ? 1 : 0;
         }
-        HIPCHK(vk::cg_update(K, c->M, cu, diag, cs, dp, nullptr, fuse, red(SL_CG, g), dc, c->st));
+        HIPCHK(vk::cg_update(K, c->M, cv, diag, cs, dp, nullptr, fuse, red(SL_CG, g), dc, c->st));
         if (c->use_comm) {
             STCHK(allreduce_dev(c, c->scal + SL_CG, (size_t)(3 * K)));
             if (fold) {
@@ -431,14 +488,22 @@
         STCHK(op_check_err(c));
         store_iters(*this, last);
         if (offer) hs->pre_made = last.pre;
+        if (offer) hs->n_made = last.pre ? 1 : 0;
+        if (offer3) {
+            hs->n_made = std::min(nrun, 2);
+            hs->pre_made = hs->n_made > 0;
+        }
         return VAMPOMI_OK;
     }
 
     vampomi_status run() {
         if (!head) STCHK(first_products());
         if (pre2) STCHK(compose_step());
+        if (J == 2) STCHK(compose_step2());
         if (head) STCHK(head_step());
         offer = pre_ok && packed && hs->pre_offer && hs->xnext && hs->axnext && !fold;
+        offer3 = offer && hs->pre3 && c->sys3_ok && hs->T2 && hs->U2;
+        if (offer3) offer = false;
         if (offer) {
             token = ++c->pre_seq;
             cu.pre_u1 = hs->U1;
@@ -446,7 +511,7 @@
             cu.pre_token = token;
         }
         CgOutcome last;
-        STCHK(cg_loop(c, a.max_iter, packed, *this, &last));
+        STCHK(cg_loop(c, a.max_iter, packed, *this, &last, &nrun));
         return finish(last);
     }
 };
@@ -531,7 +596,10 @@
 };
 
 vampomi_status pcg_run(vampomi_ctx* c, const std::vector<CgSystem*>& sys, const PcgArgs& args) {
-    if (args.hs) args.hs->used = args.hs->pre_made = args.hs->pre_used = false;
+    if (args.hs) {
+        args.hs->used = args.hs->pre_made = args.hs->pre_used = false;
+        args.hs->n_made = args.hs->n_used = 0;
+    }
     STCHK(pcg_check(c, sys, args));
     bool rec = false;
     for (const CgSystem* y : sys) rec = rec || y->W;
diff --git a/vampomi_amd/csrc/pcg.hip b/vampomi_amd/csrc/pcg.hip
--- a/vampomi_amd/csrc/pcg.hip
+++ b/vampomi_amd/csrc/pcg.hip
@@ -406,10 +406,55 @@
         u += a.gam2 * a.ab[j];
         a.AD[j] = u / a.diag;
     }
+    if (a.rz_save && blockIdx.x == 0 && threadIdx.x == 0) a.rz_save[0] = a.cs->rz[0];
     block_put_sums<1>(acc, 1, ro, (int64_t)blockIdx.x);
     red_finish(ro, 1, lds);
 }
 
+__global__ __launch_bounds__(kBlock) void pre_compose2_kernel(int64_t M, int64_t N, PreCompose2 a, RedOut ro) {
+    if (ro.gate && !*ro.gate) return;
+    if (!a.cs->active[0]) return;
+    __shared__ double lds[4];
+    const double alpha0 = a.rz_save[0] / a.dp0[0];
+    const double beta0 = a.cs->beta[0];
+    double acc[1] = {0.0};
+    const int64_t stride = (int64_t)gridDim.x * kBlock;
+    for (int64_t i = (int64_t)blockIdx.x * kBlock + threadIdx.x; i < M; i += stride) {
+        const double t1 = a.T1[i];
+        double w = a.tau * a.T2[i];
+        w += a.gam2 * t1;
+        w = w / a.diag;
+        double s = (t1 - alpha0 * w) / a.diag;
+        s = s + beta0 * (t1 / a.diag);
+        const double p1 = a.z[i] + beta0 * a.p[i];
+        double d = s * a.tau;
+        d += a.gam2 * p1;
+        a.d[i] = d;
+        if (a.S) a.S[i] = s;
+        acc[0] += d * p1;
+    }
+    for (int64_t j = (int64_t)blockIdx.x * kBlock + threadIdx.x; j < N; j += stride) {
+        const double u1 = a.U1[j];
+        double w = a.tau * a.U2[j];
+        w += a.gam2 * u1;
+        w = w / a.diag;
+        double s = (u1 - alpha0 * w) / a.diag;
+        s = s + beta0 * (u1 / a.diag);
+        double q1 = a.ar[j] / a.diag;
+        q1 = q1 + beta0 * a.q[j];
+        double u = a.tau * s;
+        u += a.gam2 * q1;
+        a.AD[j] = u;
+    }
+    block_put_sums<1>(acc, 1, ro, (int64_t)blockIdx.x);
+    red_finish(ro, 1, lds);
+}
+
+hipError_t pre_compose2(int64_t M, int64_t N, const PreCompose2& a, const RedOut& ro, hipStream_t st) {
+    hipLaunchKernelGGL(pre_compose2_kernel, dim3(red_blocks(M)), dim3(kBlock), 0, st, M, N, a, ro);
+    return hipGetLastError();
+}
+
 hipError_t pre_compose(int64_t M, int64_t N, const PreCompose& a, const RedOut& ro, hipStream_t st) {
     hipLaunchKernelGGL(pre_compose_kernel, dim3(red_blocks(M)), dim3(kBlock), 0, st, M, N, a, ro);
     return hipGetLastError();
diff --git a/vampomi_amd/csrc/run.h b/vampomi_amd/csrc/run.h
--- a/vampomi_amd/csrc/run.h
+++ b/vampomi_amd/csrc/run.h
@@ -53,6 +53,9 @@
     double* pre_t1 = nullptr;
     double* pre_u1 = nullptr;
     int pre_it = 0;
+    double* pre_t2 = nullptr;
+    double* pre_u2 = nullptr;
+    int pre_n = 0;
     double* mixw = nullptr;
     double* mixh = nullptr;
     double* mixh_dev = nullptr;
diff --git a/vampomi_amd/csrc/vamp.cpp b/vampomi_amd/csrc/vamp.cpp
--- a/vampomi_amd/csrc/vamp.cpp
+++ b/vampomi_amd/csrc/vamp.cpp
@@ -11,7 +11,7 @@
 VampRun::~VampRun() {
     if (writer) writer->drain(nullptr);
     for (double** p : {&r1, &x1, &x1p, &x1n, &x1d, &r2, &x2, &bern, &invQ, &v, &atxy, &ts, &tmpM, &atx0, &z1buf,
-                       &nb3, &nsc, &ax2, &p1, &p2, &z1h, &x1s, &x1sn, &x2s, &abern, &bern_next, &pre_t1, &pre_u1, &m_cov})
+                       &nb3, &nsc, &ax2, &p1, &p2, &z1h, &x1s, &x1sn, &x2s, &abern, &bern_next, &pre_t1, &pre_u1, &pre_t2, &pre_u2, &m_cov})
         dev_free(*p);
     for (auto& p : cgw) dev_free(p);
     dev_free(mixw);
@@ -442,6 +442,20 @@
             L.hs.pre_done = reinterpret_cast<unsigned long long*>(R.pre_u1 + ld);
             L.hs.pre_have = L.hs.abern && R.pre_it == it;
             L.hs.pre_offer = L.hs.xnext != nullptr;
+            L.hs.n_have = L.hs.pre_have ? std::max(R.pre_n, 1) : 0;
+            if (prestep_mode(c) == 3) {
+                if (!R.pre_t2) {
+                    const size_t Mx = (size_t)std::max<int64_t>(c->M, 1);
+                    STCHK(dev_alloc(&R.pre_t2, Mx));
+                    STCHK(dev_alloc(&R.pre_u2, (size_t)ld + 2));
+                    HIPCHK(hipMemsetAsync(R.pre_t2, 0, Mx * 8, c->st));
+                    HIPCHK(hipMemsetAsync(R.pre_u2, 0, ((size_t)ld + 2) * 8, c->st));
+                }
+                L.hs.pre3 = true;
+                L.hs.T2 = R.pre_t2;
+                L.hs.U2 = R.pre_u2;
+                L.hs.rz_save = R.pre_u2 + ld;
+            }
         }
     }
     vk::Prelude& pr = L.pr;
@@ -558,8 +572,9 @@
         STCHK(pcg_run(c, {&so, &sx}, pargs));
         R.hs_it = hs.xnext ? it + 1 : 0;
         R.pre_it = hs.pre_made ? it + 1 : 0;
-        c->pre_made_n += hs.pre_made ? 1 : 0;
-        c->pre_used_n += hs.pre_used ? 1 : 0;
+        R.pre_n = hs.pre_made ? std::max(hs.n_made, 1) : 0;
+        c->pre_made_n += R.pre_n;
+        c->pre_used_n += hs.pre_used ? std::max(hs.n_used, 1) : 0;
     } else if (R.fuse) {
         if (!L.arec) pargs.init = &e1;
         STCHK(pcg_run(c, {&sx, &so}, pargs));
```

Result: faster. 202.6, median of 6 (+10.5%).
